# parashardhapola/nabo

Hardware: NVIDIA B200
Metric: target_cells_mapped_per_s (higher is better)
Workload: dtype f64 (candidates: f16x2-split tcgen05, f32 accumulate)

## Files before the change

nabo_b200/csrc/exact.cu:

```cuda
#include <stdarg.h>
#include <stdio.h>

#include "common.cuh"
#include "knn_internal.cuh"
#include "select.cuh"

static thread_local char g_err[512] = "";
int nabo_set_error(int code, const char* fmt, ...) {
    va_list ap;
    va_start(ap, fmt);
    vsnprintf(g_err, sizeof(g_err), fmt, ap);
    va_end(ap);
    return code;
}
extern "C" const char* nabo_last_error(void) { return g_err; }
extern "C" int nabo_abi_version(void) { return NABO_ABI_VERSION; }
extern "C" int nabo_device_check(int* sm_count) {
    int dev = 0;
    NABO_CUDA(cudaGetDevice(&dev));
    cudaDeviceProp p;
    NABO_CUDA(cudaGetDeviceProperties(&p, dev));
    if (sm_count) *sm_count = p.multiProcessorCount;
    if (p.major != 10)
        return nabo_set_error(NABO_EUNSUPPORTED, "device %s is sm_%d%d; this library is built for sm_100a only",
                              p.name, p.major, p.minor);
    return 0;
}

template <int METRIC>
struct Pair {
    static __device__ __forceinline__ double step(double acc, double x, double y, double f) {
        if (METRIC == NABO_EUCLIDEAN) {
            double t = __dsub_rn(x, y);
            return __dadd_rn(acc, __dmul_rn(t, t));
        } else if (METRIC == NABO_MOD_CANBERRA) {
            double absx = fabs(x);
            double num = fabs(__dsub_rn(x, y));
            if (num < __dmul_rn(f, absx)) {
                double den = __dadd_rn(__dadd_rn(absx, fabs(y)), 0.01);
                return __dadd_rn(acc, __ddiv_rn(num, den));
            }
            return __dadd_rn(acc, 1.0);
        } else {
            return __dadd_rn(acc, __dmul_rn(x, y));
        }
    }
    static __device__ __forceinline__ double finish(double acc, double nq, double nr) {
        if (METRIC == NABO_EUCLIDEAN) return __dsqrt_rn(acc);
        if (METRIC == NABO_MOD_CANBERRA) return acc;
        return __dsub_rn(1.0, __ddiv_rn(acc, __dmul_rn(__dsqrt_rn(nq), __dsqrt_rn(nr))));
    }
};

__device__ __forceinline__ double seq_sqnorm(const double* v, int g) {
    double s = 0.0;
    for (int k = 0; k < g; ++k) s = __dadd_rn(s, __dmul_rn(v[k], v[k]));
    return s;
}

constexpr int TQ = 64;
constexpr int TR = 64;
constexpr int NT = 256;
constexpr int LDS_T = TQ + 2;

__device__ __forceinline__ void load_tile_kmajor(double* s, const double* __restrict__ src, int ld,
                                                 int row0, int nrows, int g, const int* row_ids, int k0 = 0) {
    for (int e = threadIdx.x; e < TQ * g; e += NT) {
        int r = e / g, k = e - r * g;
        int row = row0 + r;
        double v = 0.0;
        if (row < nrows) {
            long long rr = row_ids ? row_ids[row] : row;
            v = src[rr * (long long)ld + k0 + k];
        }
        s[k * LDS_T + r] = v;
    }
}

template <int METRIC>
__global__ void __launch_bounds__(NT) dist_tile_kernel(const double* __restrict__ x, int ldx,
                                                       const double* __restrict__ y, int ldy,
                                                       double* __restrict__ d, int ldd, int m, int n,
                                                       int g, double f) {
    extern __shared__ double smem[];
    double* xs = smem;
    double* ys = smem + (size_t)g * LDS_T;
    __shared__ double nqs[TQ], nrs[TR];
    const int q0 = blockIdx.y * TQ, r0 = blockIdx.x * TR;
    load_tile_kmajor(xs, x, ldx, q0, m, g, nullptr);
    load_tile_kmajor(ys, y, ldy, r0, n, g, nullptr);
    __syncthreads();
    if (METRIC == NABO_COSINE) {
        if (threadIdx.x < TQ) {
            double s = 0.0;
            for (int k = 0; k < g; ++k) { double v = xs[k * LDS_T + threadIdx.x]; s = __dadd_rn(s, __dmul_rn(v, v)); }
            nqs[threadIdx.x] = s;
        } else if (threadIdx.x < TQ + TR) {
            int t = threadIdx.x - TQ;
            double s = 0.0;
            for (int k = 0; k < g; ++k) { double v = ys[k * LDS_T + t]; s = __dadd_rn(s, __dmul_rn(v, v)); }
            nrs[t] = s;
        }
        __syncthreads();
    }
    const int tr = threadIdx.x & 15, tq = threadIdx.x >> 4;
    double acc[4][4];
#pragma unroll
    for (int a = 0; a < 4; ++a)
#pragma unroll
        for (int b = 0; b < 4; ++b) acc[a][b] = 0.0;
    for (int k = 0; k < g; ++k) {
        double xv[4], yv[4];
#pragma unroll
        for (int a = 0; a < 4; ++a) xv[a] = xs[k * LDS_T + tq * 4 + a];
#pragma unroll
        for (int b = 0; b < 4; ++b) yv[b] = ys[k * LDS_T + tr * 4 + b];
#pragma unroll
        for (int a = 0; a < 4; ++a)
#pragma unroll
            for (int b = 0; b < 4; ++b) acc[a][b] = Pair<METRIC>::step(acc[a][b], xv[a], yv[b], f);
    }
#pragma unroll
    for (int a = 0; a < 4; ++a) {
        int qi = q0 + tq * 4 + a;
        if (qi >= m) continue;
#pragma unroll
        for (int b = 0; b < 4; ++b) {
            int rj = r0 + tr * 4 + b;
            if (rj < n) {
                double nq = METRIC == NABO_COSINE ? nqs[tq * 4 + a] : 0.0;
                double nr = METRIC == NABO_COSINE ? nrs[tr * 4 + b] : 0.0;
                d[(long long)qi * ldd + rj] = Pair<METRIC>::finish(acc[a][b], nq, nr);
            }
        }
    }
}

template <int METRIC>
static int launch_dist_tiles(const double* x, int ldx, const double* y, int ldy, double* d, int ldd,
                             int m, int n, int g, double f, cudaStream_t s) {
    NABO_ARG(m >= 0 && n >= 0 && g >= 1, "dist: bad shape m=%d n=%d g=%d", m, n, g);
    NABO_ARG(ldx >= g && ldy >= g && ldd >= n, "dist: leading dimension smaller than row length");
    if (m == 0 || n == 0) return 0;
    NABO_ARG(x && y && d, "dist: null pointer");
    size_t smem = 2 * (size_t)g * LDS_T * sizeof(double);
    NABO_ARG(smem <= 200 * 1024, "dist: g=%d exceeds the shared-memory tile (max %d dims)", g,
             (int)(200 * 1024 / (2 * LDS_T * sizeof(double))));
    NABO_CUDA(cudaFuncSetAttribute(dist_tile_kernel<METRIC>, cudaFuncAttributeMaxDynamicSharedMemorySize, (int)smem));
    dim3 grid((n + TR - 1) / TR, (m + TQ - 1) / TQ);
    dist_tile_kernel<METRIC><<<grid, NT, smem, s>>>(x, ldx, y, ldy, d, ldd, m, n, g, f);
    NABO_LAUNCH_CHECK("dist_tile_kernel");
    return 0;
}

extern "C" int nabo_euclidean_dist(const double* x, int ldx, const double* y, int ldy, double* d, int ldd,
                                   int m, int n, int g, void* stream) {
    return launch_dist_tiles<NABO_EUCLIDEAN>(x, ldx, y, ldy, d, ldd, m, n, g, 0.0, (cudaStream_t)stream);
}
extern "C" int nabo_mod_canberra_dist(const double* x, int ldx, const double* y, int ldy, double* d, int ldd,
                                      int m, int n, int g, double f, void* stream) {
    return launch_dist_tiles<NABO_MOD_CANBERRA>(x, ldx, y, ldy, d, ldd, m, n, g, f, (cudaStream_t)stream);
}
extern "C" int nabo_cosine_dist(const double* x, int ldx, const double* y, int ldy, double* d, int ldd,
                                int m, int n, int g, void* stream) {
    return launch_dist_tiles<NABO_COSINE>(x, ldx, y, ldy, d, ldd, m, n, g, 0.0, (cudaStream_t)stream);
}

struct ExactSmem {
    double* xs;
    double* ys;
    double* bd;
    int* bi;
    double* tau_d;
    double* nq;
    double* nr;
    int* tau_i;
    int* cnt;
};

__device__ __forceinline__ ExactSmem carve_exact(double* base, int g, int cap) {
    ExactSmem s;
    s.xs = base;
    s.ys = s.xs + (size_t)g * LDS_T;
    s.bd = s.ys + (size_t)g * LDS_T;
    s.tau_d = s.bd + (size_t)TQ * cap;
    s.nq = s.tau_d + TQ;
    s.nr = s.nq + TQ;
    s.bi = (int*)(s.nr + TR);
    s.tau_i = s.bi + (size_t)TQ * cap;
    s.cnt = s.tau_i + TQ;
    return s;
}
static size_t exact_smem_bytes(int g, int cap) {
    return (2 * (size_t)g * LDS_T + (size_t)TQ * cap + 3 * TQ) * sizeof(double) +
           ((size_t)TQ * cap + 2 * TQ) * sizeof(int);
}

__device__ __forceinline__ void compact_query(const ExactSmem& s, int q, int cap, int ksel, int lane) {
    double* d = s.bd + (size_t)q * cap;
    int* ix = s.bi + (size_t)q * cap;
    int n = s.cnt[q];
    for (int t = n + lane; t < cap; t += 32) { d[t] = CUDART_INF; ix[t] = 0x7fffffff; }
    __syncwarp();
    warp_bitonic_sort(d, ix, cap, lane);
    if (lane == 0) {
        if (n >= ksel) {
            s.cnt[q] = ksel;
            s.tau_d[q] = d[ksel - 1];
            s.tau_i[q] = ix[ksel - 1];
        }
    }
    __syncwarp();
}

template <int METRIC>
__global__ void __launch_bounds__(NT, 1)
knn_exact_kernel(const double* __restrict__ q, int ldq, const double* __restrict__ r, int ldr, int n_query,
                 int n_ref, int g, int k, double f, const uint8_t* __restrict__ mask, int drop_first,
                 int idx_offset, const int* __restrict__ row_ids, const int* __restrict__ n_rows_dev,
                 int cap, int gc, const NaboExactSplit sp, int32_t* __restrict__ out_idx, double* __restrict__ out_dist,
                 const NaboRoute route) {
    extern __shared__ double smem[];
    const ExactSmem s = carve_exact(smem, gc, cap);
    const bool chunked = gc < g;
    const int nq_total = n_rows_dev ? *n_rows_dev : n_query;
    if (sp.mode == 1 && (nq_total > sp.f_max || nq_total <= sp.f_min)) return;
    if (sp.mode == 2 && nq_total <= sp.f_max) return;
    const int r_lo = sp.mode == 1 ? (int)((long long)n_ref * blockIdx.y / sp.nsplit) / TR * TR : 0;
    const int r_hi = sp.mode == 1 ? (blockIdx.y + 1 == (unsigned)sp.nsplit
                                         ? n_ref
                                         : (int)((long long)n_ref * (blockIdx.y + 1) / sp.nsplit) / TR * TR)
                                  : n_ref;
    const int q0 = blockIdx.x * TQ;
    if (q0 >= nq_total) return;
    const int ksel = k + (drop_first ? 1 : 0);
    const int lane = threadIdx.x & 31, warp = threadIdx.x >> 5;
    const int tr = threadIdx.x & 15, tq = threadIdx.x >> 4;

    if (threadIdx.x < TQ) {
        s.cnt[threadIdx.x] = 0;
        s.tau_d[threadIdx.x] = CUDART_INF;
        s.tau_i[threadIdx.x] = 0x7fffffff;
    }
    if (!chunked) {
        load_tile_kmajor(s.xs, q, ldq, q0, nq_total, g, row_ids);
        __syncthreads();
        if (METRIC == NABO_COSINE && threadIdx.x < TQ) {
            double acc = 0.0;
            for (int kk = 0; kk < g; ++kk) { double v = s.xs[kk * LDS_T + threadIdx.x]; acc = __dadd_rn(acc, __dmul_rn(v, v)); }
            s.nq[threadIdx.x] = acc;
        }
    } else if (METRIC == NABO_COSINE) {
        double acc = 0.0;
        for (int kc = 0; kc < g; kc += gc) {
            const int gn = min(gc, g - kc);
            __syncthreads();
            load_tile_kmajor(s.xs, q, ldq, q0, nq_total, gn, row_ids, kc);
            __syncthreads();
            if (threadIdx.x < TQ)
                for (int kk = 0; kk < gn; ++kk) { double v = s.xs[kk * LDS_T + threadIdx.x]; acc = __dadd_rn(acc, __dmul_rn(v, v)); }
        }
        if (threadIdx.x < TQ) s.nq[threadIdx.x] = acc;
    }

    for (int r0 = r_lo; r0 < r_hi; r0 += TR) {
        double acc[4][4];
#pragma unroll
        for (int a = 0; a < 4; ++a)
#pragma unroll
            for (int b = 0; b < 4; ++b) acc[a][b] = 0.0;
        for (int kc = 0; kc < g; kc += gc) {
            const int gn = min(gc, g - kc);
            __syncthreads();
            if (chunked) load_tile_kmajor(s.xs, q, ldq, q0, nq_total, gn, row_ids, kc);
            load_tile_kmajor(s.ys, r, ldr, r0, r_hi, gn, nullptr, kc);
            __syncthreads();
            if (METRIC == NABO_COSINE && threadIdx.x < TR) {
                double nacc = kc == 0 ? 0.0 : s.nr[threadIdx.x];
                for (int kk = 0; kk < gn; ++kk) { double v = s.ys[kk * LDS_T + threadIdx.x]; nacc = __dadd_rn(nacc, __dmul_rn(v, v)); }
                s.nr[threadIdx.x] = nacc;
            }
            if (q0 + tq * 4 < nq_total)
            for (int kk = 0; kk < gn; ++kk) {
                double xv[4], yv[4];
#pragma unroll
                for (int a = 0; a < 4; ++a) xv[a] = s.xs[kk * LDS_T + tq * 4 + a];
#pragma unroll
                for (int b = 0; b < 4; ++b) yv[b] = s.ys[kk * LDS_T + tr * 4 + b];
#pragma unroll
                for (int a = 0; a < 4; ++a)
#pragma unroll
                    for (int b = 0; b < 4; ++b) acc[a][b] = Pair<METRIC>::step(acc[a][b], xv[a], yv[b], f);
            }
        }
        if (METRIC == NABO_COSINE) __syncthreads();
#pragma unroll
        for (int a = 0; a < 4; ++a) {
            const int ql = tq * 4 + a;
            if (q0 + ql >= nq_total) continue;
            const double td = s.tau_d[ql];
            const int ti = s.tau_i[ql];
#pragma unroll
            for (int b = 0; b < 4; ++b) {
                const int j = r0 + tr * 4 + b;
                if (j >= r_hi) continue;
                double d = Pair<METRIC>::finish(acc[a][b], METRIC == NABO_COSINE ? s.nq[ql] : 0.0,
                                                METRIC == NABO_COSINE ? s.nr[tr * 4 + b] : 0.0);
                if (d != d || (mask && mask[j])) d = CUDART_INF;
                if (nabo_less(d, j, td, ti)) {
                    int pos = atomicAdd(&s.cnt[ql], 1);
                    s.bd[(size_t)ql * cap + pos] = d;
                    s.bi[(size_t)ql * cap + pos] = j;
                }
            }
        }
        __syncthreads();
        for (int ql = warp; ql < TQ; ql += NT / 32)
            if (s.cnt[ql] > cap - TR) compact_query(s, ql, cap, ksel, lane);
    }
    __syncthreads();
    for (int ql = warp; ql < TQ; ql += NT / 32) {
        const int qi = q0 + ql;
        if (qi >= nq_total) continue;
        const int n_have = s.cnt[ql];
        {
            double* d = s.bd + (size_t)ql * cap;
            int* ix = s.bi + (size_t)ql * cap;
            for (int t = n_have + lane; t < cap; t += 32) { d[t] = CUDART_INF; ix[t] = 0x7fffffff; }
            __syncwarp();
            warp_bitonic_sort(d, ix, cap, lane);
        }
        if (sp.mode == 1) {
            for (int t = lane; t < ksel; t += 32) {
                const bool have = t < n_have && t < cap;
                const size_t o = ((size_t)blockIdx.y * sp.f_max + qi) * ksel + t;
                sp.part_idx[o] = have ? s.bi[(size_t)ql * cap + t] : -1;
                sp.part_dist[o] = have ? s.bd[(size_t)ql * cap + t] : CUDART_INF;
            }
            continue;
        }
        const long long orow = row_ids ? row_ids[qi] : qi;
        int32_t* oi;
        double* od;
        nabo_route_row(route, orow, k, out_idx, out_dist, oi, od);
        const int skip = drop_first ? 1 : 0;
        for (int t = lane; t < k; t += 32) {
            int src = t + skip;
            int id = -1;
            double dv = CUDART_NAN;
            if (src < n_have && src < cap) {
                id = s.bi[(size_t)ql * cap + src];
                dv = s.bd[(size_t)ql * cap + src];
                if (mask && mask[id]) dv = CUDART_NAN;
                else if (dv == CUDART_INF) {
                    dv = CUDART_NAN;
                }
                id += idx_offset;
            }
            oi[t] = id;
            od[t] = dv;
        }
    }
}

static int exact_cap_for(int ksel) {
    int kp = nabo_next_pow2(ksel);
    int cap = 2 * kp;
    if (cap < 128) cap = 128;
    return cap;
}

__global__ void __launch_bounds__(128)
fallback_merge_kernel(const NaboExactSplit sp, const int* __restrict__ row_ids, const int* __restrict__ n_rows_dev,
                      int k, int drop_first, int idx_offset, const uint8_t* __restrict__ mask, int capp,
                      int32_t* __restrict__ out_idx, double* __restrict__ out_dist, const NaboRoute route) {
    extern __shared__ double smem[];
    const int n_rows = *n_rows_dev;
    if (n_rows > sp.f_max || n_rows <= sp.f_min) return;
    const int lane = threadIdx.x & 31, warp = threadIdx.x >> 5;
    const int qi = blockIdx.x * 4 + warp;
    if (qi >= n_rows) return;
    const int ksel = k + (drop_first ? 1 : 0);
    double* d = smem + (size_t)warp * capp;
    int* ix = (int*)(smem + (size_t)4 * capp) + (size_t)warp * capp;
    const int tot = sp.nsplit * ksel;
    int n_valid = 0;
    for (int c = lane; c < capp; c += 32) {
        double dv = CUDART_INF;
        int id = 0x7fffffff;
        if (c < tot) {
            const int sidx = c / ksel, j = c - sidx * ksel;
            const size_t o = ((size_t)sidx * sp.f_max + qi) * ksel + j;
            const int i0 = sp.part_idx[o];
            if (i0 >= 0) { id = i0; dv = sp.part_dist[o]; ++n_valid; }
        }
        d[c] = dv; ix[c] = id;
    }
    for (int o = 16; o > 0; o >>= 1) n_valid += __shfl_xor_sync(0xffffffffu, n_valid, o);
    __syncwarp();
    warp_bitonic_sort(d, ix, capp, lane);
    const long long orow = row_ids[qi];
    int32_t* oi;
    double* od;
    nabo_route_row(route, orow, k, out_idx, out_dist, oi, od);
    const int skip = drop_first ? 1 : 0;
    for (int t = lane; t < k; t += 32) {
        const int src = t + skip;
        int id = -1;
        double dv = CUDART_NAN;
        if (src < n_valid) {
            id = ix[src];
            dv = d[src];
            if (dv == CUDART_INF || (mask && mask[id])) dv = CUDART_NAN;
            id += idx_offset;
        }
        oi[t] = id;
        od[t] = dv;
    }
}

__global__ void __launch_bounds__(256)
fallback_merge_few_kernel(const NaboExactSplit sp, const int* __restrict__ row_ids, const int* __restrict__ n_rows_dev,
                          int k, int drop_first, int idx_offset, const uint8_t* __restrict__ mask, int capp,
                          int32_t* __restrict__ out_idx, double* __restrict__ out_dist, const NaboRoute route) {
    extern __shared__ double smem[];
    const int n_rows = *n_rows_dev;
    if (n_rows > sp.f_max || n_rows <= sp.f_min) return;
    const int qi = blockIdx.x;
    if (qi >= n_rows) return;
    const int ksel = k + (drop_first ? 1 : 0);
    double* d = smem;
    int* ix = (int*)(smem + capp);
    __shared__ int s_valid;
    if (threadIdx.x == 0) s_valid = 0;
    __syncthreads();
    const int tot = sp.nsplit * ksel;
    int n_valid = 0;
    for (int c = threadIdx.x; c < capp; c += blockDim.x) {
        double dv = CUDART_INF;
        int id = 0x7fffffff;
        if (c < tot) {
            const int sidx = c / ksel, j = c - sidx * ksel;
            const size_t o = ((size_t)sidx * sp.f_max + qi) * ksel + j;
            const int i0 = sp.part_idx[o];
            if (i0 >= 0) { id = i0; dv = sp.part_dist[o]; ++n_valid; }
        }
        d[c] = dv; ix[c] = id;
    }
    atomicAdd(&s_valid, n_valid);
    __syncthreads();
    for (int size = 2; size <= capp; size <<= 1)
        for (int stride = size >> 1; stride > 0; stride >>= 1) {
            for (int t = threadIdx.x; t < (capp >> 1); t += blockDim.x) {
                const int lo = 2 * t - (t & (stride - 1)), hi = lo + stride;
                const bool up = (lo & size) == 0;
                const double dl = d[lo], dh = d[hi];
                const int il = ix[lo], ih = ix[hi];
                if (up ? nabo_less(dh, ih, dl, il) : nabo_less(dl, il, dh, ih)) { d[lo] = dh; d[hi] = dl; ix[lo] = ih; ix[hi] = il; }
            }
            __syncthreads();
        }
    const long long orow = row_ids[qi];
    int32_t* oi;
    double* od;
    nabo_route_row(route, orow, k, out_idx, out_dist, oi, od);
    const int skip = drop_first ? 1 : 0;
    for (int t = threadIdx.x; t < k; t += blockDim.x) {
        const int src = t + skip;
        int id = -1;
        double dv = CUDART_NAN;
        if (src < s_valid) {
            id = ix[src];
            dv = d[src];
            if (dv == CUDART_INF || (mask && mask[id])) dv = CUDART_NAN;
            id += idx_offset;
        }
        oi[t] = id;
        od[t] = dv;
    }
}

int nabo_exact_split_count(int ksel) {
    int s = 2048 / ksel;
    return s > 48 ? 48 : (s < 1 ? 1 : s);
}
size_t nabo_exact_split_workspace(int ksel) {
    (void)ksel;
    return (size_t)2048 * NABO_FALLBACK_SPLIT_ROWS * (sizeof(int32_t) + sizeof(double)) + 512 +
           (size_t)NABO_FALLBACK_FEW_ENTRIES * NABO_FALLBACK_FEW_ROWS * (sizeof(int32_t) + sizeof(double)) + 512;
}

int nabo_knn_exact_fallback(const double* q, int ldq, const double* r, int ldr, int n_query, int n_ref, int g, int k,
                            int metric, double f, const uint8_t* mask, int drop_first, int idx_offset,
                            const int* row_ids, const int* n_rows_dev, void* split_ws, int32_t* out_idx,
                            double* out_dist, const NaboRoute& route, cudaStream_t st) {
    const int ksel = k + (drop_first ? 1 : 0);
    const bool few = n_ref >= NABO_FALLBACK_FEW_MIN_REF;
    if (few) {
        int dev = 0, sms = 148;
        cudaGetDevice(&dev);
        cudaDeviceGetAttribute(&sms, cudaDevAttrMultiProcessorCount, dev);
        NaboExactSplit sf;
        sf.mode = 1;
        sf.nsplit = NABO_FALLBACK_FEW_ENTRIES / ksel < 2 * sms ? NABO_FALLBACK_FEW_ENTRIES / ksel : 2 * sms;
        sf.f_max = NABO_FALLBACK_FEW_ROWS;
        sf.f_min = 0;
        char* base = (char*)split_ws + (size_t)2048 * NABO_FALLBACK_SPLIT_ROWS * (sizeof(int32_t) + sizeof(double)) + 512;
        sf.part_dist = (double*)base;
        sf.part_idx = (int32_t*)(sf.part_dist + (size_t)sf.nsplit * sf.f_max * ksel);
        int rc0 = nabo_knn_exact_launch_ex(q, ldq, r, ldr, NABO_FALLBACK_FEW_ROWS, n_ref, g, ksel, metric, f, mask, 0, 0,
                                           row_ids, n_rows_dev, sf, out_idx, out_dist, route, st);
        if (rc0) return rc0;
        const int cappf = nabo_next_pow2(sf.nsplit * ksel);
        const size_t smf = (size_t)cappf * (sizeof(double) + sizeof(int));
        NABO_CUDA(cudaFuncSetAttribute(fallback_merge_few_kernel, cudaFuncAttributeMaxDynamicSharedMemorySize, (int)smf));
        fallback_merge_few_kernel<<<NABO_FALLBACK_FEW_ROWS, 256, smf, st>>>(sf, row_ids, n_rows_dev, k, drop_first, idx_offset,
                                                                         mask, cappf, out_idx, out_dist, route);
        NABO_LAUNCH_CHECK("fallback_merge_few_kernel");
    }
    NaboExactSplit sp;
    sp.mode = 1;
    sp.nsplit = nabo_exact_split_count(ksel);
    sp.f_max = NABO_FALLBACK_SPLIT_ROWS;
    sp.f_min = few ? NABO_FALLBACK_FEW_ROWS : 0;
    sp.part_dist = (double*)split_ws;
    sp.part_idx = (int32_t*)(sp.part_dist + (size_t)sp.nsplit * sp.f_max * ksel);
    int rc = nabo_knn_exact_launch_ex(q, ldq, r, ldr, NABO_FALLBACK_SPLIT_ROWS, n_ref, g, ksel, metric, f, mask, 0, 0,
                                      row_ids, n_rows_dev, sp, out_idx, out_dist, route, st);
    if (rc) return rc;
    int capp = nabo_next_pow2(sp.nsplit * ksel);
    if (capp < 32) capp = 32;
    const size_t smem = (size_t)4 * capp * (sizeof(double) + sizeof(int));
    NABO_CUDA(cudaFuncSetAttribute(fallback_merge_kernel, cudaFuncAttributeMaxDynamicSharedMemorySize, (int)smem));
    fallback_merge_kernel<<<(NABO_FALLBACK_SPLIT_ROWS + 3) / 4, 128, smem, st>>>(sp, row_ids, n_rows_dev, k, drop_first,
                                                                               idx_offset, mask, capp, out_idx, out_dist,
                                                                               route);
    NABO_LAUNCH_CHECK("fallback_merge_kernel");
    sp.mode = 2;
    return nabo_knn_exact_launch_ex(q, ldq, r, ldr, n_query, n_ref, g, k, metric, f, mask, drop_first, idx_offset,
                                    row_ids, n_rows_dev, sp, out_idx, out_dist, route, st);
}

int nabo_knn_exact_launch(const double* q, int ldq, const double* r, int ldr, int n_query, int n_ref, int g,
                          int k, int metric, double f, const uint8_t* mask, int drop_first, int idx_offset,
                          const int* row_ids, const int* n_rows_dev, int32_t* out_idx, double* out_dist,
                          const NaboRoute& route, cudaStream_t st) {
    NaboExactSplit sp;
    sp.mode = 0; sp.nsplit = 1; sp.f_max = 0; sp.f_min = 0; sp.part_idx = nullptr; sp.part_dist = nullptr;
    return nabo_knn_exact_launch_ex(q, ldq, r, ldr, n_query, n_ref, g, k, metric, f, mask, drop_first, idx_offset,
                                    row_ids, n_rows_dev, sp, out_idx, out_dist, route, st);
}

int nabo_knn_exact_launch_ex(const double* q, int ldq, const double* r, int ldr, int n_query, int n_ref, int g,
                             int k, int metric, double f, const uint8_t* mask, int drop_first, int idx_offset,
                             const int* row_ids, const int* n_rows_dev, const NaboExactSplit& sp, int32_t* out_idx,
                             double* out_dist, const NaboRoute& route, cudaStream_t st) {
    const int ksel = k + (drop_first ? 1 : 0);
    NABO_ARG(k >= 1 && ksel <= 128, "knn: k=%d unsupported (1 <= k, k + drop_first <= 128)", k);
    NABO_ARG(g >= 1, "knn: g=%d", g);
    if (n_query == 0) return 0;
    const int cap = exact_cap_for(ksel);
    int gc = g;
    while (gc > 8 && exact_smem_bytes(gc, cap) > (size_t)227 * 1024) gc = (gc + 1) / 2;
    size_t smem = exact_smem_bytes(gc, cap);
    NABO_ARG(smem <= 227 * 1024, "knn: g=%d with k=%d needs %zu B of shared memory (max 232448)", g, k, smem);
    dim3 grid((n_query + TQ - 1) / TQ, sp.mode == 1 ? sp.nsplit : 1);
#define LAUNCH(M)                                                                                         \
    NABO_CUDA(cudaFuncSetAttribute(knn_exact_kernel<M>, cudaFuncAttributeMaxDynamicSharedMemorySize, (int)smem)); \
    knn_exact_kernel<M><<<grid, NT, smem, st>>>(q, ldq, r, ldr, n_query, n_ref, g, k, f, mask, drop_first, \
                                                idx_offset, row_ids, n_rows_dev, cap, gc, sp, out_idx, out_dist, route);
    if (metric == NABO_EUCLIDEAN) { LAUNCH(NABO_EUCLIDEAN) }
    else if (metric == NABO_MOD_CANBERRA) { LAUNCH(NABO_MOD_CANBERRA) }
    else if (metric == NABO_COSINE) { LAUNCH(NABO_COSINE) }
    else return nabo_set_error(NABO_EINVAL, "knn: unknown metric %d", metric);
#undef LAUNCH
    NABO_LAUNCH_CHECK("knn_exact_kernel");
    return 0;
}

__device__ __forceinline__ double cert_lower_bound(const NaboCert& c, int qi, float tau) {
    if (c.kind == NABO_CERT_LINEAR) return (double)tau - c.c_acc;
    const double sc_inv = c.scal[1], rmax = c.scal[2];
    const double qn2 = c.qn2[qi];
    const double qn = sqrt(qn2);
    const double eps = c.c_acc * (4.0 * qn * rmax + rmax * rmax + qn2);
    const double l2 = (double)tau + qn2 - eps;
    if (!(l2 > 0.0)) return 0.0;
    if (c.kind == NABO_CERT_EUCLID) {
        return sqrt(l2) * sc_inv * (1.0 - 1e-7) - (9.6e-7 * (qn + rmax) + c.abs_slack) * sc_inv;
    }
    double e = sqrt(l2) * sc_inv - 1.0e-6;
    if (!(e > 0.0)) return 0.0;
    return 0.5 * e * e * (1.0 - 1e-9);
}

template <int METRIC, int NU>
__device__ __forceinline__ void pair_rows(const double* __restrict__ x, const double* __restrict__ r, int ldr,
                                          const int* jj, int g, double f, bool vec2, double* acc) {
    const double* y[NU];
#pragma unroll
    for (int u = 0; u < NU; ++u) y[u] = r + (long long)(jj[u] >= 0 ? jj[u] : 0) * ldr;
    double a[NU];
#pragma unroll
    for (int u = 0; u < NU; ++u) a[u] = 0.0;
    int kk = 0;
    if (vec2) {
#pragma unroll 4
        for (; kk + 2 <= g; kk += 2) {
            const double x0 = x[kk], x1 = x[kk + 1];
#pragma unroll
            for (int u = 0; u < NU; ++u) {
                const double2 v = __ldg(reinterpret_cast<const double2*>(y[u] + kk));
                a[u] = Pair<METRIC>::step(a[u], x0, v.x, f);
                a[u] = Pair<METRIC>::step(a[u], x1, v.y, f);
            }
        }
    }
#pragma unroll 4
    for (; kk < g; ++kk) {
        const double xv = x[kk];
#pragma unroll
        for (int u = 0; u < NU; ++u) a[u] = Pair<METRIC>::step(a[u], xv, __ldg(y[u] + kk), f);
    }
#pragma unroll
    for (int u = 0; u < NU; ++u) acc[u] = a[u];
}

#ifdef NABO_RR_STATS
__device__ unsigned long long g_rr_stats[8];
extern "C" int nabo_dbg_rr_stats(unsigned long long* out_host, int reset) {
    cudaDeviceSynchronize();
    cudaMemcpyFromSymbol(out_host, g_rr_stats, sizeof(unsigned long long) * 8);
    if (reset) { unsigned long long z[8] = {0}; cudaMemcpyToSymbol(g_rr_stats, z, sizeof(z)); }
    return 0;
}
#endif
template <int METRIC, bool FROM_BUF>
__global__ void __launch_bounds__(128)
rerank_kernel(const double* __restrict__ q, int ldq, const double* __restrict__ r, int ldr, int n_query,
              int n_ref, int g, int k, double f, const uint8_t* __restrict__ mask, int drop_first,
              int idx_offset, const int32_t* __restrict__ cand, int n_cand, int capp, const NaboCert cert,
              int* __restrict__ fail_rows, int* __restrict__ fail_count,
              int32_t* __restrict__ out_idx, double* __restrict__ out_dist, const NaboRoute route,
              const NaboCandBuf cb, int xs_dims, bool vec2, int row0) {
    extern __shared__ double smem[];
    const int lane = threadIdx.x & 31, warp = threadIdx.x >> 5;
    const int qi = row0 + blockIdx.x * 4 + warp;
    if (qi >= n_query) return;
    int32_t* oi;
    double* od;
    nabo_route_row(route, qi, k, out_idx, out_dist, oi, od);
    double* d = smem + (size_t)warp * capp;
    int* ix = (int*)(smem + (size_t)4 * capp) + (size_t)warp * capp;
    const size_t hist_off = (size_t)6 * capp + (size_t)4 * xs_dims;
    const double* x = q + (long long)qi * ldq;
    double nq = 0.0;
    if (METRIC == NABO_COSINE) nq = seq_sqnorm(x, g);
    int nc = 0;
    float tau_q = CUDART_INF_F;
    if (FROM_BUF) {
        const int n = __ldcg(cb.cnt + qi);
        const unsigned long long* gb = cb.buf + (size_t)qi * sel::CAP;
        float fv[4];
        uint32_t kpl[4];
#pragma unroll
        for (int u = 0; u < 4; ++u) {
            const int i = u * 32 + lane;
            const unsigned long long kv = i < n ? __ldcg(gb + i) : 0ull;
            fv[u] = __uint_as_float((uint32_t)(kv >> 32));
            kpl[u] = (uint32_t)kv;
        }
        uint32_t* hist = reinterpret_cast<uint32_t*>(smem + hist_off) + warp * 256;
        int bin[4], cut_bin, kept;
        bool reach;
        sel::histogram_cut(fv, n, lane, cb.kprime, hist, bin, cut_bin, kept, reach);
        const int c_cut = reach ? (int)hist[cut_bin] : 0;
        const int need = cb.kprime - (kept - c_cut);
#ifdef NABO_RR_STATS
        if (lane == 0) {
            atomicAdd(&g_rr_stats[0], 1ull); atomicAdd(&g_rr_stats[1], (unsigned long long)(reach && c_cut > 48));
            atomicAdd(&g_rr_stats[2], (unsigned long long)c_cut); atomicAdd(&g_rr_stats[3], (unsigned long long)n);
            atomicAdd(&g_rr_stats[4], (unsigned long long)(reach ? c_cut - need : 0));
        }
#endif
        if (!reach || c_cut <= 48) {
            int rank[4] = {0, 0, 0, 0};
            if (reach && c_cut > need) {
#pragma unroll
                for (int us = 0; us < 4; ++us) {
                    unsigned mm = __ballot_sync(0xffffffffu, us * 32 + lane < n && bin[us] == cut_bin);
                    while (mm) {
                        const int src = __ffs(mm) - 1;
                        mm &= mm - 1;
                        const float sv = __shfl_sync(0xffffffffu, fv[us], src);
#pragma unroll
                        for (int u = 0; u < 4; ++u)
                            rank[u] += (sv < fv[u] || (sv == fv[u] && us * 32 + src < u * 32 + lane)) ? 1 : 0;
                    }
                }
                kept = cb.kprime;
            }
            int base = 0;
            float tmax = -CUDART_INF_F;
#pragma unroll
            for (int u = 0; u < 4; ++u) {
                const bool keep = u * 32 + lane < n && (bin[u] < cut_bin || (bin[u] == cut_bin && rank[u] < need));
                const unsigned m = __ballot_sync(0xffffffffu, keep);
                if (keep) {
                    ix[base + __popc(m & ((1u << lane) - 1u))] = (int)kpl[u];
                    tmax = fmaxf(tmax, fv[u]);
                }
                base += __popc(m);
            }
            tmax = sortable_to_float(__reduce_max_sync(0xffffffffu, float_to_sortable(tmax)));
            nc = kept;
            tau_q = reach ? tmax : __ldcg(cb.tau + qi);
        } else {
            uint32_t ks[4];
#pragma unroll
            for (int u = 0; u < 4; ++u) ks[u] = u * 32 + lane < n ? float_to_sortable(fv[u]) : 0xffffffffu;
            sel::sortn(ks, kpl, lane);
            nc = n < cb.kprime ? n : cb.kprime;
            const int e = cb.kprime - 1;
            const uint32_t ts = __shfl_sync(0xffffffffu, (e >> 5) ? ks[1] : ks[0], e & 31);
            tau_q = n >= cb.kprime ? sortable_to_float(ts) : __ldcg(cb.tau + qi);
#pragma unroll
            for (int u = 0; u < 2; ++u)
                if (u * 32 + lane < nc) ix[u * 32 + lane] = (int)kpl[u];
        }
        __syncwarp();
    } else if (cert.kind != NABO_CERT_NONE) {
        tau_q = cert.tau[qi];
    }
    double* xw = xs_dims ? smem + (size_t)4 * capp + (size_t)(4 * capp + 1) / 2 + (size_t)warp * xs_dims : nullptr;
    if (xw) {
        for (int kk = lane; kk < g; kk += 32) xw[kk] = x[kk];
        __syncwarp();
    }
    const double* xq = xw ? xw : x;
    int jj[4];
    int n_slots = 0;
    const bool scramble = (long long)n_ref * ldr * 8 > (96ll << 20);
#pragma unroll
    for (int u = 0; u < 4; ++u) {
        const int c = u * 32 + lane;
        int j = -1;
        if (u * 32 < capp) {
            if (FROM_BUF) {
                const int cpos = scramble ? ((c * 27 + 5) & (capp - 1)) : c;
                j = (u < 2 && cpos < nc) ? ix[cpos] : -1;
            }
            else j = c < n_cand ? cand[(long long)qi * n_cand + c] : -1;
        }
        if (!(j >= 0 && j < n_ref)) j = -1;
        jj[u] = j;
        if (__any_sync(0xffffffffu, j >= 0)) n_slots = u + 1;
    }
    double accs[4] = {0.0, 0.0, 0.0, 0.0};
    if (METRIC == NABO_MOD_CANBERRA) {
#pragma unroll
        for (int u = 0; u < 4; ++u)
            if (u < n_slots) pair_rows<METRIC, 1>(xq, r, ldr, jj + u, g, f, vec2, accs + u);
    } else if (n_slots == 1) pair_rows<METRIC, 1>(xq, r, ldr, jj, g, f, vec2, accs);
    else if (n_slots == 2) pair_rows<METRIC, 2>(xq, r, ldr, jj, g, f, vec2, accs);
    else if (n_slots > 2) pair_rows<METRIC, 4>(xq, r, ldr, jj, g, f, vec2, accs);
    int n_valid = 0, n_finite = 0;
    int ids[4];
#pragma unroll
    for (int u = 0; u < 4; ++u) {
        const int j = jj[u];
        double key = CUDART_INF;
        int id = 0x7fffffff;
        if (j >= 0) {
            double nr = 0.0;
            if (METRIC == NABO_COSINE) nr = seq_sqnorm(r + (long long)j * ldr, g);
            double dv = Pair<METRIC>::finish(accs[u], nq, nr);
            if (dv != dv || (mask && mask[j])) dv = CUDART_INF;
            key = dv;
            id = j;
            ++n_valid;
            n_finite += (dv < CUDART_INF);
        }
        accs[u] = key; ids[u] = id;
    }
    if (capp <= 32) {
        double d1[1] = {accs[0]};
        int i1[1] = {ids[0]};
        warp_bitonic_sort_regs<1>(d1, i1, lane);
        d[lane] = d1[0]; ix[lane] = i1[0];
    } else if (capp <= 64) {
        double d2[2] = {accs[0], accs[1]};
        int i2[2] = {ids[0], ids[1]};
        warp_bitonic_sort_regs<2>(d2, i2, lane);
#pragma unroll
        for (int u = 0; u < 2; ++u) { d[u * 32 + lane] = d2[u]; ix[u * 32 + lane] = i2[u]; }
    } else {
        warp_bitonic_sort_regs<4>(accs, ids, lane);
#pragma unroll
        for (int u = 0; u < 4; ++u) { d[u * 32 + lane] = accs[u]; ix[u * 32 + lane] = ids[u]; }
    }
    __syncwarp();
    for (int o = 16; o > 0; o >>= 1) {
        n_valid += __shfl_xor_sync(0xffffffffu, n_valid, o);
        n_finite += __shfl_xor_sync(0xffffffffu, n_finite, o);
    }
    __syncwarp();
    const int skip = drop_first ? 1 : 0;
    const int ksel = k + skip;
    for (int t = lane; t < k; t += 32) {
        int src = t + skip;
        int id = -1;
        double dv = CUDART_NAN;
        if (src < n_valid) {
            id = ix[src];
            dv = d[src];
            if (dv == CUDART_INF) dv = CUDART_NAN;
            id += idx_offset;
        }
        oi[t] = id;
        od[t] = dv;
    }
    if (cert.kind != NABO_CERT_NONE && lane == 0) {
        const float tau = tau_q;
        bool fail;
        if (tau == CUDART_INF_F) fail = n_valid < n_ref;
        else if (n_finite < ksel) fail = true;
        else fail = !(d[ksel - 1] < cert_lower_bound(cert, qi, tau));
        if (fail) fail_rows[atomicAdd(fail_count, 1)] = qi;
    }
}

int nabo_rerank_launch(const double* q, int ldq, const double* r, int ldr, int n_query, int n_ref, int g, int k,
                       int metric, double f, const uint8_t* mask, int drop_first, int idx_offset,
                       const int32_t* cand, int n_cand, const NaboCert& cert, int* fail_rows, int* fail_count,
                       int32_t* out_idx, double* out_dist, const NaboRoute& route, cudaStream_t st,
                       const NaboCandBuf* from_buf, int row0, bool dependent) {
    NABO_ARG(n_cand >= 1 && n_cand <= 128, "rerank: n_cand=%d unsupported (1..128)", n_cand);
    NABO_ARG(k >= 1 && k + (drop_first ? 1 : 0) <= n_cand, "rerank: k=%d does not fit n_cand=%d", k, n_cand);
    NABO_ARG(row0 >= 0 && row0 <= n_query, "rerank: row0=%d outside [0, %d]", row0, n_query);
    if (n_query - row0 == 0) return 0;
    int capp = nabo_next_pow2(n_cand);
    if (capp < 32) capp = 32;
    size_t smem = (size_t)4 * capp * (sizeof(double) + sizeof(int));
    const int xs_dims = g <= 1024 ? g : 0;
    smem += (size_t)4 * xs_dims * sizeof(double);
    if (from_buf) smem += (size_t)4 * 256 * sizeof(uint32_t);
    const bool vec2 = ((uintptr_t)r & 15) == 0 && (ldr & 1) == 0;
    dim3 grid((n_query - row0 + 3) / 4);
    NaboCandBuf cb;
    cb.buf = nullptr; cb.cnt = nullptr; cb.tau = nullptr; cb.kprime = 0;
    if (from_buf) {
        NABO_ARG(from_buf->kprime >= 1 && from_buf->kprime <= 64 && from_buf->kprime == n_cand,
                 "rerank: buffer mode needs K' = n_cand <= 64");
        cb = *from_buf;
    }
    cudaLaunchConfig_t cfg = {};
    cudaLaunchAttribute attr[1];
    cfg.gridDim = grid; cfg.blockDim = dim3(128); cfg.dynamicSmemBytes = smem; cfg.stream = st;
    attr[0].id = cudaLaunchAttributeProgrammaticStreamSerialization;
    attr[0].val.programmaticStreamSerializationAllowed = 1;
    cfg.attrs = attr; cfg.numAttrs = dependent ? 1 : 0;
#define LAUNCH(M)                                                                                              \
    if (from_buf)                                                                                              \
        NABO_CUDA(cudaLaunchKernelEx(&cfg, rerank_kernel<M, true>, q, ldq, r, ldr, n_query, n_ref, g, k, f, mask, \
                                     drop_first, idx_offset, cand, n_cand, capp, cert, fail_rows, fail_count,  \
                                     out_idx, out_dist, route, cb, xs_dims, vec2, row0));                      \
    else                                                                                                       \
        NABO_CUDA(cudaLaunchKernelEx(&cfg, rerank_kernel<M, false>, q, ldq, r, ldr, n_query, n_ref, g, k, f, mask, \
                                     drop_first, idx_offset, cand, n_cand, capp, cert, fail_rows, fail_count,  \
                                     out_idx, out_dist, route, cb, xs_dims, vec2, row0));
    if (metric == NABO_EUCLIDEAN) { LAUNCH(NABO_EUCLIDEAN) }
    else if (metric == NABO_MOD_CANBERRA) { LAUNCH(NABO_MOD_CANBERRA) }
    else if (metric == NABO_COSINE) { LAUNCH(NABO_COSINE) }
    else return nabo_set_error(NABO_EINVAL, "rerank: unknown metric %d", metric);
#undef LAUNCH
    NABO_LAUNCH_CHECK("rerank_kernel");
    return 0;
}

extern "C" int nabo_rerank_exact(const double* q, int ldq, const double* r, int ldr, int n_query, int n_ref,
                                 int g, int k, int metric, double dist_factor, const uint8_t* ref_mask,
                                 int drop_first, int idx_offset, const int32_t* cand, int n_cand,
                                 int32_t* out_idx, double* out_dist, void* stream) {
    NABO_ARG(q && r && cand && out_idx && out_dist, "rerank: null pointer");
    NABO_ARG(ldq >= g && ldr >= g, "rerank: leading dimension smaller than g");
    NaboCert none;
    none.kind = NABO_CERT_NONE; none.tau = nullptr; none.qn2 = nullptr; none.scal = nullptr; none.c_acc = 0.0; none.abs_slack = 0.0;
    NaboRoute plain;
    plain.n_parts = 0;
    return nabo_rerank_launch(q, ldq, r, ldr, n_query, n_ref, g, k, metric, dist_factor, ref_mask, drop_first,
                              idx_offset, cand, n_cand, none, nullptr, nullptr, out_idx, out_dist, plain,
                              (cudaStream_t)stream);
}
```

nabo_b200/csrc/fast.cu:

```cuda
#include "knn_internal.cuh"

static const double kCAcc = 1.52587890625e-05;

static size_t cb_extra_bytes(int n_query, int n_ref, int g) {
    const size_t a = nabo_cb_extra_bytes(n_ref, g), b = nabo_cbs_extra_bytes(n_query, n_ref, g);
    return a > b ? a : b;
}

size_t nabo_fast_workspace_bytes(int n_query, int n_ref, int g, int k, int metric) {
    if (metric == NABO_MOD_CANBERRA)
        return nabo_align_up((size_t)n_query * nabo_cb_kprime(k, 1) * 4 * NABO_CBS_MAX_SPLIT, 256) +
               (2 + NABO_CBS_MAX_SPLIT) * nabo_align_up((size_t)n_query * 4, 256) +
               nabo_align_up(nabo_cb_pretile_floats(n_query, g) * 4, 256) + nabo_align_up(nabo_cb_pretile_floats(n_ref, g) * 4, 256) +
               nabo_align_up(nabo_exact_split_workspace(k + 1), 256) + nabo_align_up(cb_extra_bytes(n_query, n_ref, g), 256) + 4096;
    return nabo_tc_workspace_bytes(n_query, n_ref, g, k, 1) + nabo_align_up((size_t)n_query * 4, 256) +
           nabo_align_up(nabo_exact_split_workspace(k + 1), 256) + 1024;
}

int nabo_knn_fast(const double* q, int ldq, const double* r, int ldr, int n_query, int n_ref, int g, int k,
                  int metric, double f, const uint8_t* mask, int drop_first, int idx_offset, int32_t* out_idx,
                  double* out_dist, const NaboRoute& route, void* workspace, size_t workspace_bytes,
                  int64_t* stats_host, cudaStream_t st) {
    NaboStageTimer tm(stats_host != nullptr, st);
    tm.begin();
    const bool use_tc = (metric == NABO_EUCLIDEAN || metric == NABO_COSINE) && nabo_tc_supported(g, k, drop_first) &&
                        n_ref > nabo_tc_kprime(k, drop_first);
    const bool use_cb = metric == NABO_MOD_CANBERRA && nabo_cb_supported(g, k, drop_first) &&
                        n_ref > nabo_cb_kprime(k, drop_first);
    if (use_cb) {
        if (workspace_bytes < nabo_fast_workspace_bytes(n_query, n_ref, g, k, metric))
            return nabo_set_error(NABO_EWORKSPACE, "knn: workspace too small");
        NaboArena ar(workspace, workspace_bytes);
        const int kprime = nabo_cb_kprime(k, drop_first);
        const bool sliced_ok = nabo_cbs_supported(g, k, drop_first) && f >= 1e-6;
        const int n_split = sliced_ok ? nabo_cbs_split(n_query, n_ref, k, drop_first) : 1;
        int32_t* cand = ar.take<int32_t>((size_t)n_query * kprime * n_split);
        float* tau = ar.take<float>((size_t)n_query * n_split);
        int* fail_rows = ar.take<int>(n_query);
        int* fail_count = ar.take<int>(1);
        float* qt = ar.take<float>(nabo_cb_pretile_floats(n_query, g));
        float* rt = ar.take<float>(nabo_cb_pretile_floats(n_ref, g));
        char* split_ws = ar.take<char>(nabo_exact_split_workspace(k + (drop_first ? 1 : 0)));
        char* extra = ar.take<char>(cb_extra_bytes(n_query, n_ref, g));
        if (!ar.ok) return nabo_set_error(NABO_EWORKSPACE, "knn: workspace too small");
        NABO_CUDA(cudaMemsetAsync(fail_count, 0, sizeof(int), st));
        const bool sliced = sliced_ok;
        int rc = sliced
                     ? nabo_cbs_candidates(q, ldq, r, ldr, n_query, n_ref, g, k, f, mask, drop_first, n_split, rt, extra,
                                           cb_extra_bytes(n_query, n_ref, g), cand, tau, st)
                     : nabo_cb_candidates(q, ldq, r, ldr, n_query, n_ref, g, k, f, mask, drop_first, qt, rt, extra, cand,
                                          tau, st);
        if (rc) return rc;
        if (n_split > 1) {
            rc = nabo_tau_min_launch(tau, n_query, n_split, st);
            if (rc) return rc;
        }
        tm.end(0);
        NaboCert cert;
        cert.kind = NABO_CERT_LINEAR; cert.tau = tau; cert.qn2 = nullptr; cert.scal = nullptr; cert.c_acc = nabo_cb_eps(g); cert.abs_slack = 0.0;
        rc = nabo_rerank_launch(q, ldq, r, ldr, n_query, n_ref, g, k, metric, f, mask, drop_first, idx_offset, cand,
                                kprime * n_split, cert, fail_rows, fail_count, out_idx, out_dist, route, st);
        if (rc) return rc;
        tm.end(1);
        rc = nabo_knn_exact_fallback(q, ldq, r, ldr, n_query, n_ref, g, k, metric, f, mask, drop_first, idx_offset,
                                     fail_rows, fail_count, split_ws, out_idx, out_dist, route, st);
        if (rc) return rc;
        tm.end(2);
        if (stats_host) {
            int nfail = 0;
            NABO_CUDA(cudaMemcpyAsync(&nfail, fail_count, sizeof(int), cudaMemcpyDeviceToHost, st));
            NABO_CUDA(cudaStreamSynchronize(st));
            stats_host[0] = n_query; stats_host[1] = nfail; stats_host[2] = kprime;
            stats_host[3] = sliced ? 10 : 11;
            stats_host[4] = tm.ns(0); stats_host[5] = tm.ns(1); stats_host[6] = tm.ns(2);
        }
        return 0;
    }
    if (!use_tc) {
        int rc = nabo_knn_exact_launch(q, ldq, r, ldr, n_query, n_ref, g, k, metric, f, mask, drop_first, idx_offset,
                                       nullptr, nullptr, out_idx, out_dist, route, st);
        tm.end(0);
        if (rc) return rc;
        if (stats_host) {
            NABO_CUDA(cudaStreamSynchronize(st));
            stats_host[1] = n_query;
            stats_host[3] = 1;
            stats_host[4] = tm.ns(0);
        }
        return 0;
    }
    if (workspace_bytes < nabo_fast_workspace_bytes(n_query, n_ref, g, k, metric))
        return nabo_set_error(NABO_EWORKSPACE, "knn: workspace too small (%zu < %zu)", workspace_bytes,
                              nabo_fast_workspace_bytes(n_query, n_ref, g, k, metric));
    NaboArena ar(workspace, workspace_bytes);
    int32_t* cand = nullptr;
    float* tau = nullptr;
    double *qn2 = nullptr, *scal = nullptr;
    int kprime = 0, launches = 0;
    NaboCandBuf raw;
    raw.buf = nullptr;
    int n_split = nabo_tc_split(n_query, n_ref, g);
    while (n_split > 1 && n_split * nabo_tc_kprime(k, drop_first) > 128) --n_split;
    int* fail_rows = ar.take<int>(n_query);
    int* fail_count = ar.take<int>(1);
    char* split_ws = ar.take<char>(nabo_exact_split_workspace(k + (drop_first ? 1 : 0)));
    if (!ar.ok) return nabo_set_error(NABO_EWORKSPACE, "knn: workspace too small");
    NABO_CUDA(cudaMemsetAsync(fail_count, 0, sizeof(int), st));
    NaboTailSplit tail;
    tail.rows_full = 0; tail.applies = 0;
    tail.dry = stats_host != nullptr;
    int rc = nabo_tc_candidates(q, ldq, r, ldr, n_query, n_ref, g, k, metric, mask, drop_first, &n_split, ar, &cand,
                                &kprime, &tau, &qn2, &scal, &launches, tm, st, &raw, &tail);
    if (rc) return rc;
    if (!ar.ok) return nabo_set_error(NABO_EWORKSPACE, "knn: workspace too small");
    NaboCert cert;
    cert.kind = metric == NABO_COSINE ? NABO_CERT_COSINE : NABO_CERT_EUCLID;
    cert.tau = tau; cert.qn2 = qn2; cert.scal = scal; cert.c_acc = kCAcc;
    cert.abs_slack = 2.0 * sqrt((double)g) * 5.9604644775390625e-08;
    int row0 = 0;
    if (tail.rows_full > 0) {
        rc = nabo_rerank_launch(q, ldq, r, ldr, tail.rows_full, n_ref, g, k, metric, f, mask, drop_first, idx_offset, cand,
                                kprime * n_split, cert, fail_rows, fail_count, out_idx, out_dist, route, st, &raw, 0, true);
        if (rc) return rc;
        tm.end(0);
        row0 = tail.rows_full;
    }
    launches += tail.applies;
    rc = nabo_rerank_launch(q, ldq, r, ldr, n_query, n_ref, g, k, metric, f, mask, drop_first, idx_offset, cand,
                            kprime * n_split, cert, fail_rows, fail_count, out_idx, out_dist, route, st,
                            raw.buf ? &raw : nullptr, row0);
    if (rc) return rc;
    tm.end(1);
    rc = nabo_knn_exact_fallback(q, ldq, r, ldr, n_query, n_ref, g, k, metric, f, mask, drop_first, idx_offset,
                                 fail_rows, fail_count, split_ws, out_idx, out_dist, route, st);
    if (rc) return rc;
    tm.end(2);
    if (stats_host) {
        int nfail = 0;
        NABO_CUDA(cudaMemcpyAsync(&nfail, fail_count, sizeof(int), cudaMemcpyDeviceToHost, st));
        NABO_CUDA(cudaStreamSynchronize(st));
        stats_host[0] = n_query;
        stats_host[1] = nfail;
        stats_host[2] = kprime;
        stats_host[3] = launches + 4;
        stats_host[4] = tm.ns(0);
        stats_host[5] = tm.ns(1);
        stats_host[6] = tm.ns(2);
        stats_host[7] = tm.ns(3);
    }
    return 0;
}
```

nabo_b200/csrc/knn_internal.cuh:

```cuda
#pragma once
#include "common.cuh"

#define NABO_MAX_PARTS 16
struct NaboRoute {
    int n_parts;
    int bounds[NABO_MAX_PARTS + 1];
    int32_t* idx[NABO_MAX_PARTS];
    double* dist[NABO_MAX_PARTS];
};
__device__ __forceinline__ void nabo_route_row(const NaboRoute& rt, long long row, int k, int32_t* out_idx,
                                               double* out_dist, int32_t*& ri, double*& rd) {
    if (rt.n_parts == 0) {
        ri = out_idx + row * k;
        rd = out_dist + row * k;
        return;
    }
    int p = 0;
    while (p + 1 < rt.n_parts && row >= rt.bounds[p + 1]) ++p;
    const long long local = row - rt.bounds[p];
    ri = rt.idx[p] + local * k;
    rd = rt.dist[p] + local * k;
}

#define NABO_FALLBACK_SPLIT_ROWS 2048
#define NABO_FALLBACK_FEW_ROWS 64
#define NABO_FALLBACK_FEW_ENTRIES 16384
#define NABO_FALLBACK_FEW_MIN_REF 262144
struct NaboExactSplit {
    int mode;
    int nsplit, f_max, f_min;
    int32_t* part_idx;
    double* part_dist;
};
int nabo_exact_split_count(int ksel);
size_t nabo_exact_split_workspace(int ksel);
int nabo_knn_exact_launch_ex(const double* q, int ldq, const double* r, int ldr, int n_query, int n_ref, int g,
                             int k, int metric, double f, const uint8_t* mask, int drop_first, int idx_offset,
                             const int* row_ids, const int* n_rows_dev, const NaboExactSplit& sp, int32_t* out_idx,
                             double* out_dist, const NaboRoute& route, cudaStream_t st);
int nabo_knn_exact_fallback(const double* q, int ldq, const double* r, int ldr, int n_query, int n_ref, int g, int k,
                            int metric, double f, const uint8_t* mask, int drop_first, int idx_offset,
                            const int* row_ids, const int* n_rows_dev, void* split_ws, int32_t* out_idx,
                            double* out_dist, const NaboRoute& route, cudaStream_t st);

int nabo_knn_exact_launch(const double* q, int ldq, const double* r, int ldr, int n_query, int n_ref, int g,
                          int k, int metric, double f, const uint8_t* mask, int drop_first, int idx_offset,
                          const int* row_ids, const int* n_rows_dev, int32_t* out_idx, double* out_dist,
                          const NaboRoute& route, cudaStream_t st);

#define NABO_CERT_NONE 0
#define NABO_CERT_EUCLID 1
#define NABO_CERT_COSINE 2
#define NABO_CERT_LINEAR 3
struct NaboCert {
    int kind;
    const float* tau;
    const double* qn2;
    const double* scal;
    double c_acc;
    double abs_slack;
};

struct NaboCandBuf {
    const unsigned long long* buf;
    const int* cnt;
    const float* tau;
    int kprime;
};
int nabo_rerank_launch(const double* q, int ldq, const double* r, int ldr, int n_query, int n_ref, int g, int k,
                       int metric, double f, const uint8_t* mask, int drop_first, int idx_offset,
                       const int32_t* cand, int n_cand, const NaboCert& cert, int* fail_rows, int* fail_count,
                       int32_t* out_idx, double* out_dist, const NaboRoute& route, cudaStream_t st,
                       const NaboCandBuf* from_buf = nullptr, int row0 = 0, bool dependent = false);

struct NaboTailSplit {
    int dry;
    int rows_full;
    int applies;
};

struct NaboStageTimer;
bool nabo_tc_supported(int g, int k, int drop_first);
int nabo_tc_kprime(int k, int drop_first);
size_t nabo_tc_workspace_bytes(int n_query, int n_ref, int g, int k, int drop_first);
#define NABO_TC_MAX_SPLIT 3
int nabo_tc_split(int n_query, int n_ref, int g);
int nabo_tc_candidates(const double* q, int ldq, const double* r, int ldr, int n_query, int n_ref, int g, int k,
                       int metric, const uint8_t* mask, int drop_first, int* n_split_io, NaboArena& ar, int32_t** cand_idx_out,
                       int* kprime_out, float** cert_tau_out, double** qn2_out, double** scal_out, int* launches,
                       NaboStageTimer& tm, cudaStream_t st, NaboCandBuf* raw_out = nullptr, NaboTailSplit* tail = nullptr);

bool nabo_cb_supported(int g, int k, int drop_first);
int nabo_cb_kprime(int k, int drop_first);
double nabo_cb_eps(int g);
size_t nabo_cb_pretile_floats(int n, int g);
size_t nabo_cb_extra_bytes(int n_ref, int g);
int nabo_cb_candidates(const double* q, int ldq, const double* r, int ldr, int n_query, int n_ref, int g, int k,
                       double f, const uint8_t* mask, int drop_first, float* qt, float* rt, void* extra, int32_t* cand,
                       float* tau, cudaStream_t st);

int nabo_cb_pretile_launch(const double* x, int ld, int n, int g, float* out, cudaStream_t st);
bool nabo_cbs_supported(int g, int k, int drop_first);
size_t nabo_cbs_extra_bytes(int n_query, int n_ref, int g);
#define NABO_CBS_MAX_SPLIT 3
int nabo_cbs_split(int n_query, int n_ref, int k, int drop_first);
int nabo_cbs_candidates(const double* q, int ldq, const double* r, int ldr, int n_query, int n_ref, int g, int k,
                        double f, const uint8_t* mask, int drop_first, int n_split, float* rt, void* extra,
                        size_t extra_bytes, int32_t* cand, float* tau, cudaStream_t st);
int nabo_tau_min_launch(float* tau, int n_query, int n_split, cudaStream_t st);

size_t nabo_fast_workspace_bytes(int n_query, int n_ref, int g, int k, int metric);
int nabo_knn_fast(const double* q, int ldq, const double* r, int ldr, int n_query, int n_ref, int g, int k,
                  int metric, double f, const uint8_t* mask, int drop_first, int idx_offset, int32_t* out_idx,
                  double* out_dist, const NaboRoute& route, void* workspace, size_t workspace_bytes,
                  int64_t* stats_host, cudaStream_t st);

struct NaboStageTimer {
    static constexpr int MAXS = 4;
    bool on;
    cudaStream_t st;
    cudaEvent_t start;
    cudaEvent_t stop[MAXS];
    int prev[MAXS];
    bool used[MAXS];
    int last;
    NaboStageTimer(bool enable, cudaStream_t s) : on(enable), st(s), last(-1) {
        for (int i = 0; i < MAXS; ++i) { prev[i] = -1; used[i] = false; }
        if (on) {
            cudaEventCreate(&start);
            for (int i = 0; i < MAXS; ++i) cudaEventCreate(&stop[i]);
        }
    }
    ~NaboStageTimer() {
        if (on) {
            cudaEventDestroy(start);
            for (int i = 0; i < MAXS; ++i) cudaEventDestroy(stop[i]);
        }
    }
    void begin() { if (on) cudaEventRecord(start, st); }
    void end(int i) {
        if (!on) return;
        cudaEventRecord(stop[i], st);
        used[i] = true;
        prev[i] = last;
        last = i;
    }
    long long ns(int i) {
        if (!on || !used[i]) return 0;
        float ms = 0.f;
        cudaEventElapsedTime(&ms, prev[i] < 0 ? start : stop[prev[i]], stop[i]);
        return (long long)((double)ms * 1e6);
    }
};
```

nabo_b200/csrc/select.cuh:

```cuda
#pragma once
#include "common.cuh"

namespace sel {

constexpr int CAP = 128;
constexpr int KPL = CAP / 32;

__device__ __forceinline__ unsigned long long make_key(float score, uint32_t col) {
    return ((unsigned long long)__float_as_uint(score) << 32) | col;
}

__device__ __forceinline__ void cex(uint32_t& s0, uint32_t& p0, uint32_t& s1, uint32_t& p1, bool up) {
    const bool sw = up ? (s1 < s0) : (s0 < s1);
    if (sw) { uint32_t t = s0; s0 = s1; s1 = t; t = p0; p0 = p1; p1 = t; }
}

__device__ __forceinline__ void sortn(uint32_t (&s)[KPL], uint32_t (&pl)[KPL], int lane) {
#pragma unroll
    for (int size = 2; size <= 32 * KPL; size <<= 1) {
#pragma unroll
        for (int stride = size >> 1; stride > 0; stride >>= 1) {
            if (stride >= 32) {
                const int du = stride >> 5;
#pragma unroll
                for (int u = 0; u < KPL; ++u) {
                    if ((u & du) == 0) {
                        const bool up = (((u * 32) & size) == 0);
                        cex(s[u], pl[u], s[u | du], pl[u | du], up);
                    }
                }
            } else {
#pragma unroll
                for (int u = 0; u < KPL; ++u) {
                    const int i = u * 32 + lane;
                    const uint32_t os = __shfl_xor_sync(0xffffffffu, s[u], stride);
                    const uint32_t op = __shfl_xor_sync(0xffffffffu, pl[u], stride);
                    const bool up = ((i & size) == 0);
                    const bool lower = ((lane & stride) == 0);
                    const bool take_min = (up == lower);
                    const bool other = take_min ? (os < s[u]) : (s[u] < os);
                    if (other) { s[u] = os; pl[u] = op; }
                }
            }
        }
    }
}

__device__ __forceinline__ void compact_sort_inline(unsigned long long* gbuf, int n, int lane, int kprime,
                                                    uint32_t (&s)[KPL], uint32_t (&pl)[KPL], int& nc, float& nt) {
    __syncwarp();
#pragma unroll
    for (int u = 0; u < KPL; ++u) {
        const int i = u * 32 + lane;
        const unsigned long long kv = i < n ? __ldcg(gbuf + i) : 0ull;
        s[u] = i < n ? float_to_sortable(__uint_as_float((uint32_t)(kv >> 32))) : 0xffffffffu;
        pl[u] = (uint32_t)kv;
    }
    sortn(s, pl, lane);
    nc = n < kprime ? n : kprime;
#pragma unroll
    for (int u = 0; u < KPL; ++u) {
        const int i = u * 32 + lane;
        if (i < nc) gbuf[i] = ((unsigned long long)__float_as_uint(sortable_to_float(s[u])) << 32) | pl[u];
    }
    const int e = kprime - 1;
    uint32_t ts = s[0];
#pragma unroll
    for (int u = 1; u < KPL; ++u)
        if ((e >> 5) == u) ts = s[u];
    ts = __shfl_sync(0xffffffffu, ts, e & 31);
    nt = n >= kprime ? sortable_to_float(ts) : CUDART_INF_F;
    __syncwarp();
}

static __device__ __noinline__ void compact_sort(unsigned long long* gbuf, int n, int lane, int kprime, int& nc, float& nt) {
    uint32_t s[KPL], pl[KPL];
    compact_sort_inline(gbuf, n, lane, kprime, s, pl, nc, nt);
}

static __device__ __noinline__ void compact_select(unsigned long long* gbuf, int n, int lane, int kprime, int max_keep,
                                            uint32_t* hist, int& nc, float& nt) {
    __syncwarp();
    float fv[KPL];
    uint32_t pl[KPL];
    float flo = CUDART_INF_F, fhi = -CUDART_INF_F;
#pragma unroll
    for (int u = 0; u < KPL; ++u) {
        const int i = u * 32 + lane;
        const unsigned long long kv = i < n ? __ldcg(gbuf + i) : 0ull;
        fv[u] = __uint_as_float((uint32_t)(kv >> 32));
        pl[u] = (uint32_t)kv;
        if (i < n) { flo = fminf(flo, fv[u]); fhi = fmaxf(fhi, fv[u]); }
    }
    flo = sortable_to_float(__reduce_min_sync(0xffffffffu, float_to_sortable(flo)));
    fhi = sortable_to_float(__reduce_max_sync(0xffffffffu, float_to_sortable(fhi)));
    reinterpret_cast<uint4*>(hist)[lane * 2] = make_uint4(0, 0, 0, 0);
    reinterpret_cast<uint4*>(hist)[lane * 2 + 1] = make_uint4(0, 0, 0, 0);
    __syncwarp();
    const float range = fhi - flo;
    const float scale = range > 0.f ? 255.999f / range : 0.f;
    int bin[KPL];
#pragma unroll
    for (int u = 0; u < KPL; ++u) {
        const int i = u * 32 + lane;
        bin[u] = max(0, min(255, (int)((fv[u] - flo) * scale)));
        if (i < n) atomicAdd(&hist[bin[u]], 1u);
    }
    __syncwarp();
    const uint4 h0 = reinterpret_cast<const uint4*>(hist)[lane * 2];
    const uint4 h1 = reinterpret_cast<const uint4*>(hist)[lane * 2 + 1];
    const uint32_t c[8] = {h0.x, h0.y, h0.z, h0.w, h1.x, h1.y, h1.z, h1.w};
    uint32_t mine = 0;
#pragma unroll
    for (int e = 0; e < 8; ++e) mine += c[e];
    uint32_t incl = mine;
#pragma unroll
    for (int o = 1; o < 32; o <<= 1) {
        const uint32_t v = __shfl_up_sync(0xffffffffu, incl, o);
        if (lane >= o) incl += v;
    }
    const unsigned reach = __ballot_sync(0xffffffffu, incl >= (uint32_t)kprime);
    int cut_bin = 255;
    uint32_t kept = (uint32_t)n;
    if (reach) {
        const int owner = __ffs(reach) - 1;
        uint32_t run = incl - mine;
        int b = 7;
        uint32_t k_at = 0;
        bool found = false;
#pragma unroll
        for (int e = 0; e < 8; ++e) {
            run += c[e];
            if (!found && run >= (uint32_t)kprime) { found = true; b = e; k_at = run; }
        }
        cut_bin = __shfl_sync(0xffffffffu, lane * 8 + b, owner);
        kept = __shfl_sync(0xffffffffu, k_at, owner);
    }
    if ((int)kept > max_keep) {
        compact_sort(gbuf, n, lane, kprime, nc, nt);
        return;
    }
    uint32_t base = 0;
    float tmax = -CUDART_INF_F;
#pragma unroll
    for (int u = 0; u < KPL; ++u) {
        const int i = u * 32 + lane;
        const bool keep = i < n && bin[u] <= cut_bin;
        const unsigned m = __ballot_sync(0xffffffffu, keep);
        if (keep) {
            gbuf[base + __popc(m & ((1u << lane) - 1u))] = ((unsigned long long)__float_as_uint(fv[u]) << 32) | pl[u];
            tmax = fmaxf(tmax, fv[u]);
        }
        base += __popc(m);
    }
    tmax = sortable_to_float(__reduce_max_sync(0xffffffffu, float_to_sortable(tmax)));
    nc = (int)kept;
    nt = reach ? tmax : CUDART_INF_F;
    __syncwarp();
}

__device__ __forceinline__ void histogram_cut(const float (&fv)[KPL], int n, int lane, int kprime, uint32_t* hist,
                                              int (&bin)[KPL], int& cut_bin, int& kept, bool& reach_out) {
    float flo = CUDART_INF_F, fhi = -CUDART_INF_F;
#pragma unroll
    for (int u = 0; u < KPL; ++u)
        if (u * 32 + lane < n) { flo = fminf(flo, fv[u]); fhi = fmaxf(fhi, fv[u]); }
    flo = sortable_to_float(__reduce_min_sync(0xffffffffu, float_to_sortable(flo)));
    fhi = sortable_to_float(__reduce_max_sync(0xffffffffu, float_to_sortable(fhi)));
    reinterpret_cast<uint4*>(hist)[lane * 2] = make_uint4(0, 0, 0, 0);
    reinterpret_cast<uint4*>(hist)[lane * 2 + 1] = make_uint4(0, 0, 0, 0);
    __syncwarp();
    const float range = fhi - flo;
    const float scale = range > 0.f ? 255.999f / range : 0.f;
#pragma unroll
    for (int u = 0; u < KPL; ++u) {
        bin[u] = max(0, min(255, (int)((fv[u] - flo) * scale)));
        if (u * 32 + lane < n) atomicAdd(&hist[bin[u]], 1u);
    }
    __syncwarp();
    const uint4 h0 = reinterpret_cast<const uint4*>(hist)[lane * 2];
    const uint4 h1 = reinterpret_cast<const uint4*>(hist)[lane * 2 + 1];
    const uint32_t c[8] = {h0.x, h0.y, h0.z, h0.w, h1.x, h1.y, h1.z, h1.w};
    uint32_t mine = 0;
#pragma unroll
    for (int e = 0; e < 8; ++e) mine += c[e];
    uint32_t incl = mine;
#pragma unroll
    for (int o = 1; o < 32; o <<= 1) {
        const uint32_t v = __shfl_up_sync(0xffffffffu, incl, o);
        if (lane >= o) incl += v;
    }
    const unsigned reach = __ballot_sync(0xffffffffu, incl >= (uint32_t)kprime);
    cut_bin = 255;
    kept = n;
    reach_out = reach != 0;
    if (reach) {
        const int owner = __ffs(reach) - 1;
        uint32_t run = incl - mine;
        int b = 7;
        uint32_t k_at = 0;
        bool found = false;
#pragma unroll
        for (int e = 0; e < 8; ++e) {
            run += c[e];
            if (!found && run >= (uint32_t)kprime) { found = true; b = e; k_at = run; }
        }
        cut_bin = __shfl_sync(0xffffffffu, lane * 8 + b, owner);
        kept = (int)__shfl_sync(0xffffffffu, k_at, owner);
    }
    __syncwarp();
}

}
```

nabo_b200/csrc/tc_candidates.cu:

```cuda
#include "common.cuh"
#include "knn_internal.cuh"
#include "ptx.cuh"
#include "select.cuh"

#include <cuda_fp16.h>

namespace tc {

constexpr int TILE = 128;
constexpr int NTHREADS = 512;
constexpr int MAX_G = 128;
constexpr int PRODUCER_WARP = 12;
constexpr int MMA_WARP = 13;
constexpr int TMEM_WARP = 12;
constexpr int KPL = 4;
constexpr int CAP = 32 * KPL;
static_assert(CAP == sel::CAP, "the fused re-rank (exact.cu) reads the candidate buffers with sel::CAP keys per query");
constexpr int CHUNK = 32;
constexpr int MAX_KPRIME = 96;
constexpr int SLEEP_NS = 2000;
constexpr int NACC = 4;
constexpr int MAX_STAGES = 4;
constexpr uint32_t KSTEP_BYTES = TILE * 16 * 2;

__host__ __device__ inline int kp_for(int g) { return (3 * g + 3 + 15) / 16 * 16; }
__host__ __device__ inline size_t tile_bytes(int kp) { return (size_t)TILE * kp * 2; }

struct SmemPlan {
    int nq;
    int slab;
    int stages;
    size_t stage_bytes;
    size_t a_off, b_off, sort_off, bar_off, total;
};
inline SmemPlan plan_smem(int g) {
    const int kp = kp_for(g);
    const size_t bars = 512;
    const size_t budget = 227 * 1024 - 1024;
    auto room = [&](int nq) {
        const size_t used = nq * tile_bytes(kp) + (size_t)4 * nq * 256 * 4 + bars;
        return budget > used ? budget - used : (size_t)0;
    };
    SmemPlan p;
    p.nq = 3;
    p.slab = 0;
    p.stage_bytes = tile_bytes(kp);
    p.stages = (int)(room(3) / p.stage_bytes);
    if (p.stages > MAX_STAGES) p.stages = MAX_STAGES;
    if (p.stages < 2) {
        p.nq = 2;
        p.stages = 0;
        for (int slab = 4; slab >= 2 && g <= MAX_G; slab /= 2) {
            const size_t sb = (size_t)slab * KSTEP_BYTES;
            int st = (int)(room(2) / sb);
            if (st > MAX_STAGES) st = MAX_STAGES;
            if (st >= 2 && st * sb > p.stages * p.stage_bytes) { p.slab = slab; p.stages = st; p.stage_bytes = sb; }
        }
    }
    const size_t a = p.nq * tile_bytes(kp);
    p.a_off = 0;
    p.b_off = a;
    p.sort_off = a + (size_t)p.stages * p.stage_bytes;
    p.bar_off = p.sort_off + (size_t)4 * p.nq * 256 * 4;
    p.total = p.bar_off + bars;
    return p;
}

__global__ void __launch_bounds__(256)
norms_kernel(const double* __restrict__ x, int ld, int n, int g, double* __restrict__ norms2,
             unsigned int* __restrict__ maxn2_bits) {
    int row = blockIdx.x * blockDim.x + threadIdx.x;
    float mine = 0.f;
    if (row < n) {
        const double* p = x + (long long)row * ld;
        double s = 0.0;
        for (int k = 0; k < g; ++k) s = fma(p[k], p[k], s);
        norms2[row] = s;
        if (isfinite(s)) mine = __double2float_ru(s);
    }
    for (int o = 16; o > 0; o >>= 1) mine = fmaxf(mine, __shfl_xor_sync(0xffffffffu, mine, o));
    if ((threadIdx.x & 31) == 0 && mine > 0.f) atomicMax(maxn2_bits, __float_as_uint(mine));
}

__global__ void scale_kernel(const unsigned int* __restrict__ maxq_bits, const unsigned int* __restrict__ maxr_bits,
                             int cosine, double* __restrict__ scal) {
    double sc = 1.0, rmax;
    if (cosine) {
        sc = 32.0;
        rmax = 32.0 * (1.0 + 1e-6);
    } else {
        float mq = __uint_as_float(*maxq_bits), mr = __uint_as_float(*maxr_bits);
        double mx = sqrt((double)fmaxf(mq, mr));
        if (mx > 0.0 && isfinite(mx)) {
            int e;
            frexp(mx, &e);
            sc = ldexp(1.0, 6 - e);
        }
        rmax = sqrt((double)__uint_as_float(*maxr_bits)) * sc * (1.0 + 1e-6);
    }
    scal[0] = sc;
    scal[1] = 1.0 / sc;
    scal[2] = rmax;
    scal[3] = cosine ? 1.0 : 0.0;
}

constexpr int PACK_SPLIT = 4;
template <bool IS_QUERY>
__global__ void __launch_bounds__(TILE * PACK_SPLIT)
pack_kernel(const double* __restrict__ x, int ld, int n, int g, int kp, const double* __restrict__ norms2,
            const double* __restrict__ scal, const uint8_t* __restrict__ mask, __half* __restrict__ out,
            double* __restrict__ qn2_out) {
    __shared__ double part[PACK_SPLIT][TILE];
    const int r = threadIdx.x & (TILE - 1);
    const int c = threadIdx.x / TILE;
    const long long row = (long long)blockIdx.x * TILE + r;
    __half* tile = out + (size_t)blockIdx.x * TILE * kp;
    const bool live = row < n;
    const double sc = scal[0];
    const bool cosine = scal[3] != 0.0;
    double mul = sc;
    bool dead = false;
    if (live && cosine) {
        double nn = sqrt(norms2[row]);
        if (nn > 0.0 && isfinite(nn)) mul = sc / nn; else { mul = 0.0; dead = true; }
    }
    if (live && !IS_QUERY && mask && mask[row]) dead = true;
    if (!live && !IS_QUERY) dead = true;
    const double* p = x + (live ? row : 0) * (long long)ld;
    const int nchunks = kp / 8;
    auto chunk = [&](int kc, double& n2, double n2_row) {
        __align__(16) __half h[8];
#pragma unroll
        for (int e = 0; e < 8; ++e) {
            const int col = kc * 8 + e;
            __half v = __float2half(0.f);
            if (live && col < 3 * g) {
                const int seg = col / g, k = col - seg * g;
                const double xv = p[k] * mul;
                const __half hi = __double2half(xv);
                const __half lo = __double2half(xv - (double)__half2float(hi));
                if (seg == 0) { const double t = (double)__half2float(hi) + (double)__half2float(lo); n2 = fma(t, t, n2); }
                if (IS_QUERY) {
                    const __half src = seg == 2 ? lo : hi;
                    v = __float2half(-2.0f * __half2float(src));
                } else {
                    v = seg == 1 ? lo : hi;
                }
            } else if (live && col < 3 * g + 3) {
                if (IS_QUERY) v = __float2half(1.0f);
            }
            h[e] = v;
        }
        if (!IS_QUERY && (live || dead) && 3 * g + 3 > kc * 8 && 3 * g < kc * 8 + 8) {
            double rem = dead ? 60000.0 : n2_row;
            for (int t = 0; t < 3; ++t) {
                const int col = 3 * g + t;
                const __half piece = __double2half(rem);
                rem -= (double)__half2float(piece);
                if (dead && t > 0) { if (col >= kc * 8 && col < kc * 8 + 8) h[col - kc * 8] = __float2half(0.f); continue; }
                if (col >= kc * 8 && col < kc * 8 + 8) h[col - kc * 8] = piece;
            }
        }
        *reinterpret_cast<uint4*>(reinterpret_cast<char*>(tile) + (size_t)kc * (TILE * 16) + (r >> 3) * 128 + (r & 7) * 16) =
            *reinterpret_cast<const uint4*>(h);
    };
    const int norm_lo = (3 * g) / 8, norm_hi = (3 * g + 2) / 8;
    double n2 = 0.0;
    for (int kc = c; kc < nchunks; kc += PACK_SPLIT) {
        if (!IS_QUERY && kc >= norm_lo && kc <= norm_hi) continue;
        chunk(kc, n2, 0.0);
    }
    if (!IS_QUERY) {
        for (int kc = norm_lo + c; kc <= norm_hi && kc < nchunks; kc += PACK_SPLIT)
            for (int e = 0; e < 8; ++e) {
                const int col = kc * 8 + e;
                if (live && col < g) {
                    const double xv = p[col] * mul;
                    const __half hi = __double2half(xv);
                    const __half lo = __double2half(xv - (double)__half2float(hi));
                    const double t = (double)__half2float(hi) + (double)__half2float(lo);
                    n2 = fma(t, t, n2);
                }
            }
    }
    part[c][r] = n2;
    __syncthreads();
    double n2_row = part[0][r];
#pragma unroll
    for (int i = 1; i < PACK_SPLIT; ++i) n2_row += part[i][r];
    if (!IS_QUERY) {
        for (int kc = norm_lo + c; kc <= norm_hi && kc < nchunks; kc += PACK_SPLIT) {
            double unused = 0.0;
            chunk(kc, unused, n2_row);
        }
    }
    if (IS_QUERY && c == 0 && live && qn2_out) qn2_out[row] = n2_row;
}

struct Params {
    const __half* qa;
    const __half* rb;
    int n_query, n_ref, kp, n_items, n_rtiles, stages, kprime, kc_out, soft;
    int signal_round;
    int n_split;
    unsigned long long* cand_buf;
    int* cand_cnt;
    float* cand_tau;
    int32_t* cand_idx;
    float* cert_tau;
    size_t a_off, b_off, sort_off, bar_off;
};

struct Barriers {
    uint64_t a_full, a_empty;
    uint64_t b_full[MAX_STAGES], b_empty[MAX_STAGES];
    uint64_t acc_full[NACC], acc_empty[NACC];
    uint32_t tmem_base;
};

using namespace sel;

#ifdef NABO_TC_STATS
__device__ unsigned long long g_tc_stats[12];
#define TC_STAT(i, v) (tc_loc[i] += (unsigned long long)(v))
#define TC_CLK(var) const long long var = clock64()
#define TC_CLK_ADD(i, t0) (tc_loc[i] += (unsigned long long)(clock64() - (t0)))
#define TC_DECL unsigned long long tc_loc[12] = {0, 0, 0, 0, 0, 0, 0, 0, 0, 0, 0, 0}
#define TC_FLUSH do { if ((threadIdx.x & 31) == 0) for (int i_ = 0; i_ < 12; ++i_) { if (tc_loc[i_]) atomicAdd(&g_tc_stats[i_], tc_loc[i_]); tc_loc[i_] = 0; } } while (0)
#define TC_ARG , unsigned long long (&tc_loc)[12]
#define TC_PASS , tc_loc
#else
#define TC_STAT(i, v)
#define TC_CLK(var)
#define TC_CLK_ADD(i, t0)
#define TC_DECL
#define TC_FLUSH
#define TC_ARG
#define TC_PASS
#endif

__device__ __forceinline__ void filter_chunk(const uint32_t (&vr)[32], uint32_t col0, float tau,
                                             unsigned long long* mybuf, int& cnt TC_ARG) {
    float v[32];
#pragma unroll
    for (int i = 0; i < 32; ++i) v[i] = __uint_as_float(vr[i]);
    float g4[4];
#pragma unroll
    for (int gi = 0; gi < 4; ++gi) {
        const float a = ptx::min3(v[8 * gi], v[8 * gi + 1], v[8 * gi + 2]);
        const float b = ptx::min3(v[8 * gi + 3], v[8 * gi + 4], v[8 * gi + 5]);
        g4[gi] = ptx::min3(a, b, fminf(v[8 * gi + 6], v[8 * gi + 7]));
    }
    const float m = fminf(fminf(g4[0], g4[1]), fminf(g4[2], g4[3]));
#ifdef NABO_TC_STATS
    {
        const unsigned hb = __ballot_sync(0xffffffffu, m < tau);
        if ((threadIdx.x & 31) == 0) { TC_STAT(0, 1); if (hb) { TC_STAT(1, 1); TC_STAT(2, __popc(hb)); } }
        int na = 0;
        for (int i = 0; i < 32; ++i) na += v[i] < tau;
        for (int o = 16; o > 0; o >>= 1) na += __shfl_xor_sync(0xffffffffu, na, o);
        if ((threadIdx.x & 31) == 0) TC_STAT(3, na);
    }
#endif
    if (m < tau) {
#pragma unroll
        for (int gi = 0; gi < 4; ++gi) {
            if (g4[gi] < tau) {
#pragma unroll
                for (int i = 0; i < 8; ++i) {
                    if (v[8 * gi + i] < tau) {
                        NABO_DEV_ASSERT(cnt >= 0 && cnt < CAP);
                        mybuf[cnt] = make_key(v[8 * gi + i], col0 + 8 * gi + i);
                        ++cnt;
                    }
                }
            }
        }
    }
}

template <bool SPLIT>
__device__ __forceinline__ bool work_piece(const Params& p, int c, int r, int& slot, int& qitem, int& j0, int& j1) {
    slot = c + r * (int)gridDim.x;
    if (!SPLIT) {
        if (slot >= p.n_items) return false;
        qitem = slot; j0 = 0; j1 = p.n_rtiles;
        return true;
    }
    if (slot >= p.n_items * p.n_split) return false;
    qitem = slot / p.n_split;
    const int seg = slot - qitem * p.n_split;
    j0 = (int)((long long)p.n_rtiles * seg / p.n_split);
    j1 = (int)((long long)p.n_rtiles * (seg + 1) / p.n_split);
    return true;
}

template <int KSTEPS, bool SPLIT, int NQ = 3, int SLAB = 0>
__global__ void __launch_bounds__(NTHREADS, 1) candidates_kernel(const Params p) {
    static_assert(NQ * 4 <= PRODUCER_WARP && (SLAB == 0 || KSTEPS == 0), "tile plan");
    constexpr int N_EPI_WARPS = 4 * NQ;
    extern __shared__ __align__(1024) uint8_t smem[];
    Barriers* bars = reinterpret_cast<Barriers*>(smem + p.bar_off);
    const int warp = threadIdx.x >> 5, lane = threadIdx.x & 31;
    const int ksteps = p.kp / 16;
    const uint32_t a_tile_bytes = (uint32_t)tile_bytes(p.kp);
    const int nslab = SLAB ? (ksteps + SLAB - 1) / SLAB : 1;
    const uint32_t stage_bytes = SLAB ? SLAB * KSTEP_BYTES : a_tile_bytes;

    if (threadIdx.x == 0) {
        ptx::mbar_init(&bars->a_full, 1);
        ptx::mbar_init(&bars->a_empty, 1);
        for (int s = 0; s < MAX_STAGES; ++s) { ptx::mbar_init(&bars->b_full[s], 1); ptx::mbar_init(&bars->b_empty[s], 1); }
        for (int q = 0; q < NACC; ++q) { ptx::mbar_init(&bars->acc_full[q], 1); ptx::mbar_init(&bars->acc_empty[q], 4); }
        ptx::fence_barrier_init();
    }
    if (warp == TMEM_WARP) ptx::tmem_alloc(&bars->tmem_base, 512);
    ptx::tc_fence_before();
    __syncthreads();
    ptx::tc_fence_after();
    const uint32_t tmem_base = bars->tmem_base;

    if (warp == PRODUCER_WARP) {
        if (lane == 0) {
            uint32_t t = 0, it = 0;
            for (int wr = 0;; ++wr, ++it) {
                int w, item, j0, j1;
                if (!work_piece<SPLIT>(p, blockIdx.x, wr, w, item, j0, j1)) break;
                ptx::mbar_wait_hint(&bars->a_empty, (it & 1) ^ 1, SLEEP_NS);
                ptx::mbar_arrive_expect_tx(&bars->a_full, NQ * a_tile_bytes);
                for (int q = 0; q < NQ; ++q) {
                    const char* src = reinterpret_cast<const char*>(p.qa) + (size_t)(item * NQ + q) * a_tile_bytes;
                    char* dst = reinterpret_cast<char*>(smem + p.a_off) + (size_t)q * a_tile_bytes;
                    for (uint32_t o = 0; o < a_tile_bytes; o += 8192)
                        ptx::bulk_g2s(dst + o, src + o, min(8192u, a_tile_bytes - o), &bars->a_full);
                }
                for (int j = j0; j < j1; ++j)
                    for (int sl = 0; sl < nslab; ++sl, ++t) {
                        const uint32_t s = t % p.stages, use = t / p.stages;
                        const uint32_t off = sl * stage_bytes, bytes = min(stage_bytes, a_tile_bytes - off);
                        ptx::mbar_wait_hint(&bars->b_empty[s], (use & 1) ^ 1, SLEEP_NS);
                        ptx::mbar_arrive_expect_tx(&bars->b_full[s], bytes);
                        const char* src = reinterpret_cast<const char*>(p.rb) + (size_t)j * a_tile_bytes + off;
                        char* dst = reinterpret_cast<char*>(smem + p.b_off) + (size_t)s * stage_bytes;
                        for (uint32_t o = 0; o < bytes; o += 8192)
                            ptx::bulk_g2s(dst + o, src + o, min(8192u, bytes - o), &bars->b_full[s]);
                    }
            }
        }
    } else if (warp == MMA_WARP) {
        {
            const uint32_t idesc = ptx::make_idesc_f16(TILE, TILE);
            const uint32_t lbo = TILE * 16, sbo = 128;
            const uint64_t ad0 = ptx::make_smem_desc(ptx::smem_u32(smem + p.a_off), lbo, sbo);
            const uint64_t bd0 = ptx::make_smem_desc(ptx::smem_u32(smem + p.b_off), lbo, sbo);
            uint32_t t = 0, it = 0, n = 0;
            for (int wr = 0;; ++wr, ++it) {
                int w, item, j0, j1;
                if (!work_piece<SPLIT>(p, blockIdx.x, wr, w, item, j0, j1)) break;
                ptx::mbar_wait(&bars->a_full, it & 1);
                for (int j = j0; j < j1; ++j, n += NQ, ++t)
                    for (int sl = 0; sl < nslab; ++sl) {
                        const uint32_t u = t * nslab + sl, s = u % p.stages, use = u / p.stages;
                        ptx::mbar_wait(&bars->b_full[s], use & 1);
                        const uint64_t bd1 = bd0 + (uint64_t)((s * stage_bytes) >> 4);
                        const int k0 = sl * SLAB;
#pragma unroll
                        for (int q = 0; q < NQ; ++q) {
                            const uint32_t job = n + q, buf = job & 3;
                            if (sl == 0) {
                                ptx::mbar_wait(&bars->acc_empty[buf], ((job >> 2) & 1) ^ 1);
                                ptx::tc_fence_after();
                            }
                            const uint32_t d_tmem = tmem_base + buf * TILE;
                            const uint64_t ad1 = ad0 + (uint64_t)((q * a_tile_bytes + k0 * KSTEP_BYTES) >> 4);
                            if (ptx::elect_one()) {
                                if (SLAB > 0) {
#pragma unroll
                                    for (int ks = 0; ks < SLAB; ++ks)
                                        if (k0 + ks < ksteps)
                                            ptx::mma_f16_ss(d_tmem, ad1 + ks * ((2 * lbo) >> 4), bd1 + ks * ((2 * lbo) >> 4),
                                                            idesc, k0 + ks > 0 ? 1u : 0u);
                                } else if (KSTEPS > 0) {
#pragma unroll
                                    for (int ks = 0; ks < KSTEPS; ++ks)
                                        ptx::mma_f16_ss(d_tmem, ad1 + ks * ((2 * lbo) >> 4), bd1 + ks * ((2 * lbo) >> 4), idesc,
                                                        ks > 0 ? 1u : 0u);
                                } else {
                                    for (int ks = 0; ks < ksteps; ++ks)
                                        ptx::mma_f16_ss(d_tmem, ad1 + ks * ((2 * lbo) >> 4), bd1 + ks * ((2 * lbo) >> 4), idesc,
                                                        ks > 0 ? 1u : 0u);
                                }
                                if (sl == nslab - 1) ptx::mma_commit(&bars->acc_full[buf]);
                                if (q == NQ - 1) {
                                    ptx::mma_commit(&bars->b_empty[s]);
                                    if (j == j1 - 1 && sl == nslab - 1) ptx::mma_commit(&bars->a_empty);
                                }
                            }
                            __syncwarp();
                        }
                    }
            }
        }
    } else if (warp < N_EPI_WARPS) {
        const int q = warp >> 2;
        const int quarter = warp & 3;
        const int row = quarter * 32 + lane;
        const int slot = q * TILE + row;
        const uint32_t tlane0 = tmem_base + ((uint32_t)(quarter * 32) << 16);
        uint32_t t = 0;
        uint32_t* hist = reinterpret_cast<uint32_t*>(smem + p.sort_off) + (size_t)warp * 256;
        TC_DECL;
        for (int wr = 0;; ++wr) {
            int w, item, j0, j1;
            if (!work_piece<SPLIT>(p, blockIdx.x, wr, w, item, j0, j1)) break;
            unsigned long long* mybuf = p.cand_buf + ((size_t)w * NQ * TILE + slot) * CAP;
            float tau = CUDART_INF_F;
            int cnt = 0;
            TC_CLK(t_item);
            for (int j = j0; j < j1; ++j, ++t) {
                const uint32_t job = t * NQ + q, buf = job & 3, acc_par = (job >> 2) & 1;
                const uint32_t taddr0 = tlane0 + buf * TILE;
                TC_CLK(t_w);
                ptx::mbar_wait(&bars->acc_full[buf], acc_par);
                ptx::tc_fence_after();
                TC_CLK_ADD(7, t_w);
                NABO_DEV_ASSERT(j >= 0 && j < p.n_rtiles);
                auto compact_over = [&](int lim) {
                    unsigned need = __ballot_sync(0xffffffffu, cnt > lim);
                    TC_CLK(t_c);
                    while (need) {
                        const int src = __ffs(need) - 1;
                        need &= need - 1;
                        unsigned long long* gb = reinterpret_cast<unsigned long long*>(
                            __shfl_sync(0xffffffffu, (unsigned long long)mybuf, src));
                        const int n = __shfl_sync(0xffffffffu, cnt, src);
                        int nc;
                        float nt;
                        compact_select(gb, n, lane, p.kprime, p.soft - 8, hist, nc, nt);
                        if (lane == src) { cnt = nc; tau = nt; }
                        if (lane == 0) TC_STAT(4, 1);
                    }
                    TC_CLK_ADD(5, t_c);
                };
#pragma unroll 1
                for (int c = 0; c < TILE / CHUNK; ++c) {
                    uint32_t vr[32];
                    TC_CLK(t_l);
                    ptx::tmem_ld_32x32(taddr0 + c * CHUNK, vr);
                    ptx::tmem_ld_wait();
                    TC_CLK_ADD(8, t_l);
                    if (c == TILE / CHUNK - 1) {
                        ptx::tc_fence_before();
                        __syncwarp();
                        if (lane == 0) ptx::mbar_arrive(&bars->acc_empty[buf]);
                    }
                    TC_CLK(t_f);
                    filter_chunk(vr, (uint32_t)(j * TILE + c * CHUNK), tau, mybuf, cnt TC_PASS);
                    TC_CLK_ADD(6, t_f);
                    compact_over(c == TILE / CHUNK - 1 ? p.soft : CAP - CHUNK);
                }
            }
            TC_CLK(t_e);
            p.cand_cnt[(size_t)w * NQ * TILE + slot] = cnt;
            p.cand_tau[(size_t)w * NQ * TILE + slot] = tau;
            TC_CLK_ADD(9, t_e);
            TC_CLK_ADD(10, t_item);
            TC_FLUSH;
            if (!SPLIT && p.signal_round == wr + 1) {
                __threadfence();
                asm volatile("bar.sync 1, %0;" ::"n"(N_EPI_WARPS * 32) : "memory");
                if (threadIdx.x == 0) asm volatile("griddepcontrol.launch_dependents;" ::: "memory");
            }
        }
    }
    ptx::tc_fence_before();
    __syncthreads();
    if (warp == TMEM_WARP) ptx::tmem_dealloc(tmem_base, 512);
}

template <int NQ>
__global__ void __launch_bounds__(256)
emit_kernel(const Params p) {
    const int lane = threadIdx.x & 31;
    const long long wq = (long long)blockIdx.x * 8 + (threadIdx.x >> 5);
    if (wq >= (long long)p.n_items * p.n_split * NQ * TILE) return;
    const int w = (int)(wq / (NQ * TILE)), slot = (int)(wq - (long long)w * NQ * TILE);
    const int item = w / p.n_split, seg = w - item * p.n_split;
    const long long qg = (long long)item * NQ * TILE + slot;
    if (qg >= p.n_query) return;
    const int n = p.cand_cnt[wq];
    const float old_tau = p.cand_tau[wq];
    NABO_DEV_ASSERT(n >= 0 && n <= CAP);
    uint32_t ks[KPL], kpl[KPL];
    int nc;
    float nt;
    compact_sort_inline(p.cand_buf + (size_t)wq * CAP, n, lane, p.kprime, ks, kpl, nc, nt);
#pragma unroll
    for (int u = 0; u < 4; ++u) {
        const int i = u * 32 + lane;
        if (i < p.kc_out) {
            int32_t id = -1;
            if (i < nc && kpl[u] < (uint32_t)p.n_ref) id = (int32_t)kpl[u];
            p.cand_idx[(qg * p.n_split + seg) * p.kc_out + i] = id;
        }
    }
    if (lane == 0) p.cert_tau[(long long)seg * p.n_query + qg] = n >= p.kprime ? nt : old_tau;
}

}

bool nabo_tc_supported(int g, int k, int drop_first) {
    if (g < 1 || g > tc::MAX_G) return false;
    const tc::SmemPlan pl = tc::plan_smem(g);
    const int ksel = k + (drop_first ? 1 : 0);
    return pl.stages >= 2 && ksel + 8 <= tc::MAX_KPRIME;
}

int nabo_tc_kprime(int k, int drop_first) {
    const int ksel = k + (drop_first ? 1 : 0);
    int kprime = ksel + (ksel / 4 > 8 ? ksel / 4 : 8);
    if (kprime > tc::MAX_KPRIME) kprime = tc::MAX_KPRIME;
    return kprime;
}

static int tc_grid(int n_items) {
    int dev = 0, sms = 148;
    cudaGetDevice(&dev);
    cudaDeviceGetAttribute(&sms, cudaDevAttrMultiProcessorCount, dev);
    return n_items < sms ? n_items : sms;
}

int nabo_tc_split(int n_query, int n_ref, int g) {
    const int nq = tc::plan_smem(g).nq;
    const int n_items = (n_query + nq * tc::TILE - 1) / (nq * tc::TILE);
    const int n_rtiles = (n_ref + tc::TILE - 1) / tc::TILE;
    int s = n_items > 0 ? tc_grid(1 << 30) / n_items : 1;
    if (s > NABO_TC_MAX_SPLIT) s = NABO_TC_MAX_SPLIT;
    while (s > 1 && n_rtiles / s < 32) --s;
    return s < 1 ? 1 : s;
}

__global__ void tau_min_kernel(float* __restrict__ tau, int n_query, int n_split) {
    const int i = blockIdx.x * blockDim.x + threadIdx.x;
    if (i >= n_query) return;
    float t = tau[i];
    for (int s = 1; s < n_split; ++s) t = fminf(t, tau[(size_t)s * n_query + i]);
    tau[i] = t;
}

int nabo_tau_min_launch(float* tau, int n_query, int n_split, cudaStream_t st) {
    tau_min_kernel<<<(n_query + 255) / 256, 256, 0, st>>>(tau, n_query, n_split);
    NABO_LAUNCH_CHECK("tau_min_kernel");
    return 0;
}

size_t nabo_tc_workspace_bytes(int n_query, int n_ref, int g, int k, int drop_first) {
    const int kp = tc::kp_for(g);
    const size_t tb = tc::tile_bytes(kp);
    const int nq = tc::plan_smem(g).nq;
    const int n_items = (n_query + nq * tc::TILE - 1) / (nq * tc::TILE);
    const int n_rtiles = (n_ref + tc::TILE - 1) / tc::TILE;
    const int kprime = nabo_tc_kprime(k, drop_first);
    size_t b = 0;
    b += nabo_align_up((size_t)n_items * nq * tb, 256);
    b += nabo_align_up((size_t)n_rtiles * tb, 256);
    b += nabo_align_up((size_t)n_query * 8, 256) * 2;
    b += nabo_align_up((size_t)n_ref * 8, 256);
    b += nabo_align_up((size_t)n_items * NABO_TC_MAX_SPLIT * nq * tc::TILE * (tc::CAP * 8 + 8), 256) + 512;
    b += nabo_align_up((size_t)n_query * kprime * 4 * NABO_TC_MAX_SPLIT, 256);
    b += nabo_align_up((size_t)n_query * 4 * NABO_TC_MAX_SPLIT, 256) + nabo_align_up((size_t)n_query * 4, 256);
    b += 4096;
    return b;
}

int nabo_tc_candidates(const double* q, int ldq, const double* r, int ldr, int n_query, int n_ref, int g, int k,
                       int metric, const uint8_t* mask, int drop_first, int* n_split_io, NaboArena& ar, int32_t** cand_idx_out,
                       int* kprime_out, float** cert_tau_out, double** qn2_out, double** scal_out, int* launches,
                       NaboStageTimer& tm, cudaStream_t st, NaboCandBuf* raw_out, NaboTailSplit* tail) {
    int n_split = *n_split_io;
    const int kp = tc::kp_for(g);
    const tc::SmemPlan pl = tc::plan_smem(g);
    const size_t tb = tc::tile_bytes(kp);
    const int n_items = (n_query + pl.nq * tc::TILE - 1) / (pl.nq * tc::TILE);
    const int n_qtiles = n_items * pl.nq;
    const int n_rtiles = (n_ref + tc::TILE - 1) / tc::TILE;
    const int kprime = nabo_tc_kprime(k, drop_first);
    if (n_split < 1 || n_split > NABO_TC_MAX_SPLIT) n_split = 1;
    const int grid = tc_grid(n_items * n_split);

    __half* qa = (__half*)ar.take<char>((size_t)n_qtiles * tb);
    __half* rb = (__half*)ar.take<char>((size_t)n_rtiles * tb);
    double* qnorm = ar.take<double>(n_query);
    double* qn2 = ar.take<double>(n_query);
    double* rnorm = ar.take<double>(n_ref);
    const size_t n_slots = (size_t)n_items * n_split * pl.nq * tc::TILE;
    unsigned long long* cbuf = ar.take<unsigned long long>(n_slots * tc::CAP);
    int* ccnt = ar.take<int>(n_slots);
    float* ctau = ar.take<float>(n_slots);
    int32_t* cand = ar.take<int32_t>((size_t)n_query * kprime * n_split);
    float* tau = ar.take<float>((size_t)n_query * n_split);
    double* scal = ar.take<double>(4);
    unsigned int* maxbits = ar.take<unsigned int>(2);
    if (!ar.ok) return nabo_set_error(NABO_EWORKSPACE, "knn: workspace too small for the tensor-core pass");

    NABO_CUDA(cudaMemsetAsync(maxbits, 0, 2 * sizeof(unsigned int), st));
    tc::norms_kernel<<<(n_query + 255) / 256, 256, 0, st>>>(q, ldq, n_query, g, qnorm, maxbits);
    tc::norms_kernel<<<(n_ref + 255) / 256, 256, 0, st>>>(r, ldr, n_ref, g, rnorm, maxbits + 1);
    tc::scale_kernel<<<1, 1, 0, st>>>(maxbits, maxbits + 1, metric == NABO_COSINE ? 1 : 0, scal);
    tc::pack_kernel<true><<<n_qtiles, tc::TILE * tc::PACK_SPLIT, 0, st>>>(q, ldq, n_query, g, kp, qnorm, scal, nullptr, qa, qn2);
    tc::pack_kernel<false><<<n_rtiles, tc::TILE * tc::PACK_SPLIT, 0, st>>>(r, ldr, n_ref, g, kp, rnorm, scal, mask, rb, nullptr);
    NABO_LAUNCH_CHECK("tc pack kernels");
    tm.end(3);

    tc::Params p;
    p.qa = qa; p.rb = rb;
    p.n_query = n_query; p.n_ref = n_ref; p.kp = kp; p.n_items = n_items; p.n_rtiles = n_rtiles;
    p.stages = pl.stages; p.kprime = kprime; p.kc_out = kprime; p.n_split = n_split;
    p.cand_buf = cbuf; p.cand_cnt = ccnt; p.cand_tau = ctau; p.cand_idx = cand; p.cert_tau = tau;
    p.a_off = pl.a_off; p.b_off = pl.b_off; p.sort_off = pl.sort_off; p.bar_off = pl.bar_off;
    p.soft = tc::CAP - tc::CHUNK - 16 > kprime ? tc::CAP - tc::CHUNK - 16 : kprime;
    const bool fused = raw_out && n_split == 1 && kprime <= 64;
    const int rem_items = n_items % grid;
    const bool tail_applies = tail && fused && n_items > grid && rem_items > 0 && grid - rem_items >= 16;
    const bool overlap = tail_applies && !tail->dry;
    p.signal_round = overlap ? n_items / grid : 0;
    if (tail) {
        tail->applies = tail_applies ? 1 : 0;
        tail->rows_full = overlap ? (n_items - rem_items) * pl.nq * tc::TILE : 0;
    }
#define NABO_TC_LAUNCH1(KS, SPLIT, NQ, SLAB)                                                                       \
    do {                                                                                                           \
        NABO_CUDA(cudaFuncSetAttribute(tc::candidates_kernel<KS, SPLIT, NQ, SLAB>,                                 \
                                       cudaFuncAttributeMaxDynamicSharedMemorySize, (int)pl.total));               \
        tc::candidates_kernel<KS, SPLIT, NQ, SLAB><<<grid, tc::NTHREADS, pl.total, st>>>(p);                       \
    } while (0)
#define NABO_TC_LAUNCH(KS, NQ, SLAB)                                                                               \
    do {                                                                                                           \
        if (n_split > 1) NABO_TC_LAUNCH1(KS, true, NQ, SLAB);                                                      \
        else NABO_TC_LAUNCH1(KS, false, NQ, SLAB);                                                                 \
    } while (0)
    if (pl.stages < 2) return nabo_set_error(NABO_EUNSUPPORTED, "knn: g=%d outside the tensor-core tile plans", g);
    if (pl.nq == 2) {
        if (pl.slab == 4) NABO_TC_LAUNCH(0, 2, 4);
        else NABO_TC_LAUNCH(0, 2, 2);
    } else if (kp == 160) NABO_TC_LAUNCH(10, 3, 0);
    else if (kp == 80) NABO_TC_LAUNCH(5, 3, 0);
    else NABO_TC_LAUNCH(0, 3, 0);
#undef NABO_TC_LAUNCH1
#undef NABO_TC_LAUNCH
    NABO_LAUNCH_CHECK("candidates_kernel");
    if (!overlap) tm.end(0);
    if (fused) {
        raw_out->buf = cbuf; raw_out->cnt = ccnt; raw_out->tau = ctau; raw_out->kprime = kprime;
        *cand_idx_out = cand; *kprime_out = kprime; *cert_tau_out = tau; *qn2_out = qn2; *scal_out = scal;
        *launches += 6;
        *n_split_io = 1;
        return 0;
    }
    if (raw_out) raw_out->buf = nullptr;
    if (pl.nq == 2) tc::emit_kernel<2><<<(unsigned)((n_slots + 7) / 8), 256, 0, st>>>(p);
    else tc::emit_kernel<3><<<(unsigned)((n_slots + 7) / 8), 256, 0, st>>>(p);
    NABO_LAUNCH_CHECK("emit_kernel");
    *launches += 1;
    if (n_split > 1) {
        int rc = nabo_tau_min_launch(tau, n_query, n_split, st);
        if (rc) return rc;
        *launches += 1;
    }
    *n_split_io = n_split;
    *cand_idx_out = cand; *kprime_out = kprime; *cert_tau_out = tau; *qn2_out = qn2; *scal_out = scal;
    *launches += 6;
    return 0;
}

#ifdef NABO_TC_STATS
extern "C" int nabo_dbg_tc_stats(unsigned long long* out_host, int reset) {
    cudaDeviceSynchronize();
    cudaMemcpyFromSymbol(out_host, tc::g_tc_stats, sizeof(unsigned long long) * 12);
    if (reset) { unsigned long long z[12] = {0}; cudaMemcpyToSymbol(tc::g_tc_stats, z, sizeof(z)); }
    return 0;
}
#endif

extern "C" int nabo_knn_candidates_width(int k, int drop_first) { return nabo_tc_kprime(k, drop_first); }

extern "C" size_t nabo_knn_candidates_workspace_bytes(int n_query, int n_ref, int g, int k, int drop_first) {
    return nabo_tc_workspace_bytes(n_query, n_ref, g, k, drop_first);
}

extern "C" int nabo_knn_candidates(const double* q, int ldq, const double* r, int ldr, int n_query, int n_ref, int g,
                                   int k, int metric, const uint8_t* ref_mask, int drop_first, int32_t* out_cand,
                                   float* out_tau, double* out_qn2, double* out_scal, void* workspace,
                                   size_t workspace_bytes, void* stream) {
    cudaStream_t st = (cudaStream_t)stream;
    NABO_ARG(metric == NABO_EUCLIDEAN || metric == NABO_COSINE, "candidates: metric %d has no tensor-core pass", metric);
    NABO_ARG(n_query >= 1 && n_ref >= 1 && ldq >= g && ldr >= g, "candidates: bad sizes");
    NABO_ARG(q && r && out_cand && out_tau, "candidates: null pointer");
    if (!nabo_tc_supported(g, k, drop_first))
        return nabo_set_error(NABO_EUNSUPPORTED, "candidates: g=%d k=%d outside the tensor-core tile plan", g, k);
    NaboArena ar(workspace, workspace_bytes);
    NaboStageTimer tm(false, st);
    int32_t* cand = nullptr;
    float* tau = nullptr;
    double *qn2 = nullptr, *scal = nullptr;
    int kprime = 0, launches = 0;
    int one_list = 0;
    int rc = nabo_tc_candidates(q, ldq, r, ldr, n_query, n_ref, g, k, metric, ref_mask, drop_first, &one_list, ar, &cand,
                                &kprime, &tau, &qn2, &scal, &launches, tm, st);
    if (rc) return rc;
    NABO_CUDA(cudaMemcpyAsync(out_cand, cand, sizeof(int32_t) * (size_t)n_query * kprime, cudaMemcpyDeviceToDevice, st));
    NABO_CUDA(cudaMemcpyAsync(out_tau, tau, sizeof(float) * (size_t)n_query, cudaMemcpyDeviceToDevice, st));
    if (out_qn2) NABO_CUDA(cudaMemcpyAsync(out_qn2, qn2, sizeof(double) * (size_t)n_query, cudaMemcpyDeviceToDevice, st));
    if (out_scal) NABO_CUDA(cudaMemcpyAsync(out_scal, scal, sizeof(double) * 4, cudaMemcpyDeviceToDevice, st));
    return 0;
}
```

Measured before the change: 22.99 million.

## Split only the tail wave of query items across SMs and merge pieces in rerank

Replaces the old uniform n_split of every query item with a schedule in which full waves of items run unsplit. Only the remainder items (fewer than the SM count) are split into reference-tile ranges spread over all SMs. Rerank then unions up to three candidate pieces per split row, using a shared threshold and a histogram cut. This targets the idle SMs in the last wave and removes the emit and tau-min kernels in the fused path. The cost is more complex scheduling, extra workspace, a memset, and a fallback to failed rows when the union overflows.

```diff
diff --git a/nabo_b200/csrc/exact.cu b/nabo_b200/csrc/exact.cu
--- a/nabo_b200/csrc/exact.cu
+++ b/nabo_b200/csrc/exact.cu
@@ -635,6 +635,76 @@
     return 0;
 }
 #endif
+__device__ __forceinline__ int split_union(const NaboCandBuf& cb, int qi, int lane, uint32_t* hist, float (&fv)[4],
+                                           uint32_t (&kpl)[4], float& tf) {
+    const int np = cb.pieces[qi / cb.rows_per_item];
+    const uint32_t ts = cb.shared_tau[qi];
+    tf = ts >= float_to_sortable(CUDART_INF_F) ? CUDART_INF_F : sortable_to_float(ts);
+    auto key_at = [&](int pc, int u, int& n_pc) {
+        const size_t row = (size_t)pc * cb.plane + qi;
+        n_pc = cb.cnt[row];
+        const int i = u * 32 + lane;
+        return i < n_pc ? cb.buf[row * sel::CAP + i] : 0ull;
+    };
+    int m = 0;
+    float flo = CUDART_INF_F, fhi = -CUDART_INF_F;
+    for (int pc = 0; pc < np; ++pc)
+#pragma unroll
+        for (int u = 0; u < 4; ++u) {
+            int n_pc;
+            const unsigned long long kv = key_at(pc, u, n_pc);
+            const float f = __uint_as_float((uint32_t)(kv >> 32));
+            if (u * 32 + lane < n_pc && f < tf) { ++m; flo = fminf(flo, f); fhi = fmaxf(fhi, f); }
+        }
+    m = __reduce_add_sync(0xffffffffu, m);
+    int cut_bin = 255;
+    float scale = 0.f;
+    if (m > sel::CAP) {
+        flo = sortable_to_float(__reduce_min_sync(0xffffffffu, float_to_sortable(flo)));
+        fhi = sortable_to_float(__reduce_max_sync(0xffffffffu, float_to_sortable(fhi)));
+        reinterpret_cast<uint4*>(hist)[lane * 2] = make_uint4(0, 0, 0, 0);
+        reinterpret_cast<uint4*>(hist)[lane * 2 + 1] = make_uint4(0, 0, 0, 0);
+        __syncwarp();
+        scale = fhi > flo ? 255.999f / (fhi - flo) : 0.f;
+        for (int pc = 0; pc < np; ++pc)
+#pragma unroll
+            for (int u = 0; u < 4; ++u) {
+                int n_pc;
+                const float f = __uint_as_float((uint32_t)(key_at(pc, u, n_pc) >> 32));
+                if (u * 32 + lane < n_pc && f < tf) atomicAdd(&hist[max(0, min(255, (int)((f - flo) * scale)))], 1u);
+            }
+        __syncwarp();
+        int kept;
+        sel::hist_cut(hist, m, lane, cb.kprime, cut_bin, kept);
+        __syncwarp();
+        if (kept > sel::CAP) return -1;
+    }
+    unsigned long long* stage = reinterpret_cast<unsigned long long*>(hist);
+    int base = 0;
+    for (int pc = 0; pc < np; ++pc)
+#pragma unroll
+        for (int u = 0; u < 4; ++u) {
+            int n_pc;
+            const unsigned long long kv = key_at(pc, u, n_pc);
+            const float f = __uint_as_float((uint32_t)(kv >> 32));
+            const bool keep = u * 32 + lane < n_pc && f < tf &&
+                              (m <= sel::CAP || max(0, min(255, (int)((f - flo) * scale))) <= cut_bin);
+            const unsigned mk = __ballot_sync(0xffffffffu, keep);
+            if (keep) stage[base + __popc(mk & ((1u << lane) - 1u))] = kv;
+            base += __popc(mk);
+        }
+    __syncwarp();
+#pragma unroll
+    for (int u = 0; u < 4; ++u) {
+        const int i = u * 32 + lane;
+        const unsigned long long kv = i < base ? stage[i] : 0ull;
+        fv[u] = __uint_as_float((uint32_t)(kv >> 32));
+        kpl[u] = (uint32_t)kv;
+    }
+    __syncwarp();
+    return base;
+}
+
 template <int METRIC, bool FROM_BUF>
 __global__ void __launch_bounds__(128)
 rerank_kernel(const double* __restrict__ q, int ldq, const double* __restrict__ r, int ldr, int n_query,
@@ -659,18 +729,28 @@
     int nc = 0;
     float tau_q = CUDART_INF_F;
     if (FROM_BUF) {
-        const int n = __ldcg(cb.cnt + qi);
-        const unsigned long long* gb = cb.buf + (size_t)qi * sel::CAP;
-        float fv[4];
+        uint32_t* hist = reinterpret_cast<uint32_t*>(smem + hist_off) + warp * 256;
+        const bool split_row = qi >= cb.split_row0;
+        float fv[4], tau_rest = CUDART_INF_F;
         uint32_t kpl[4];
-#pragma unroll
-        for (int u = 0; u < 4; ++u) {
-            const int i = u * 32 + lane;
-            const unsigned long long kv = i < n ? __ldcg(gb + i) : 0ull;
-            fv[u] = __uint_as_float((uint32_t)(kv >> 32));
-            kpl[u] = (uint32_t)kv;
-        }
-        uint32_t* hist = reinterpret_cast<uint32_t*>(smem + hist_off) + warp * 256;
+        int n;
+        if (!split_row) {
+            n = __ldcg(cb.cnt + qi);
+            const unsigned long long* gb = cb.buf + (size_t)qi * sel::CAP;
+#pragma unroll
+            for (int u = 0; u < 4; ++u) {
+                const int i = u * 32 + lane;
+                const unsigned long long kv = i < n ? __ldcg(gb + i) : 0ull;
+                fv[u] = __uint_as_float((uint32_t)(kv >> 32));
+                kpl[u] = (uint32_t)kv;
+            }
+        } else {
+            n = split_union(cb, qi, lane, hist, fv, kpl, tau_rest);
+            if (n < 0) {
+                if (lane == 0) fail_rows[atomicAdd(fail_count, 1)] = qi;
+                return;
+            }
+        }
         int bin[4], cut_bin, kept;
         bool reach;
         sel::histogram_cut(fv, n, lane, cb.kprime, hist, bin, cut_bin, kept, reach);
@@ -714,7 +794,7 @@
             }
             tmax = sortable_to_float(__reduce_max_sync(0xffffffffu, float_to_sortable(tmax)));
             nc = kept;
-            tau_q = reach ? tmax : __ldcg(cb.tau + qi);
+            tau_q = reach ? tmax : split_row ? tau_rest : __ldcg(cb.tau + qi);
         } else {
             uint32_t ks[4];
 #pragma unroll
@@ -723,7 +803,7 @@
             nc = n < cb.kprime ? n : cb.kprime;
             const int e = cb.kprime - 1;
             const uint32_t ts = __shfl_sync(0xffffffffu, (e >> 5) ? ks[1] : ks[0], e & 31);
-            tau_q = n >= cb.kprime ? sortable_to_float(ts) : __ldcg(cb.tau + qi);
+            tau_q = n >= cb.kprime ? sortable_to_float(ts) : split_row ? tau_rest : __ldcg(cb.tau + qi);
 #pragma unroll
             for (int u = 0; u < 2; ++u)
                 if (u * 32 + lane < nc) ix[u * 32 + lane] = (int)kpl[u];
@@ -848,7 +928,8 @@
     const bool vec2 = ((uintptr_t)r & 15) == 0 && (ldr & 1) == 0;
     dim3 grid((n_query - row0 + 3) / 4);
     NaboCandBuf cb;
-    cb.buf = nullptr; cb.cnt = nullptr; cb.tau = nullptr; cb.kprime = 0;
+    cb.buf = nullptr; cb.cnt = nullptr; cb.tau = nullptr; cb.kprime = 0; cb.split_row0 = n_query; cb.rows_per_item = 1;
+    cb.plane = 0; cb.pieces = nullptr; cb.shared_tau = nullptr;
     if (from_buf) {
         NABO_ARG(from_buf->kprime >= 1 && from_buf->kprime <= 64 && from_buf->kprime == n_cand,
                  "rerank: buffer mode needs K' = n_cand <= 64");
diff --git a/nabo_b200/csrc/fast.cu b/nabo_b200/csrc/fast.cu
--- a/nabo_b200/csrc/fast.cu
+++ b/nabo_b200/csrc/fast.cu
@@ -99,8 +99,6 @@
     int kprime = 0, launches = 0;
     NaboCandBuf raw;
     raw.buf = nullptr;
-    int n_split = nabo_tc_split(n_query, n_ref, g);
-    while (n_split > 1 && n_split * nabo_tc_kprime(k, drop_first) > 128) --n_split;
     int* fail_rows = ar.take<int>(n_query);
     int* fail_count = ar.take<int>(1);
     char* split_ws = ar.take<char>(nabo_exact_split_workspace(k + (drop_first ? 1 : 0)));
@@ -109,8 +107,8 @@
     NaboTailSplit tail;
     tail.rows_full = 0; tail.applies = 0;
     tail.dry = stats_host != nullptr;
-    int rc = nabo_tc_candidates(q, ldq, r, ldr, n_query, n_ref, g, k, metric, mask, drop_first, &n_split, ar, &cand,
-                                &kprime, &tau, &qn2, &scal, &launches, tm, st, &raw, &tail);
+    int rc = nabo_tc_candidates(q, ldq, r, ldr, n_query, n_ref, g, k, metric, mask, drop_first, ar, &cand, &kprime, &tau,
+                                &qn2, &scal, &launches, tm, st, &raw, &tail);
     if (rc) return rc;
     if (!ar.ok) return nabo_set_error(NABO_EWORKSPACE, "knn: workspace too small");
     NaboCert cert;
@@ -120,14 +118,14 @@
     int row0 = 0;
     if (tail.rows_full > 0) {
         rc = nabo_rerank_launch(q, ldq, r, ldr, tail.rows_full, n_ref, g, k, metric, f, mask, drop_first, idx_offset, cand,
-                                kprime * n_split, cert, fail_rows, fail_count, out_idx, out_dist, route, st, &raw, 0, true);
+                                kprime, cert, fail_rows, fail_count, out_idx, out_dist, route, st, &raw, 0, true);
         if (rc) return rc;
         tm.end(0);
         row0 = tail.rows_full;
     }
     launches += tail.applies;
     rc = nabo_rerank_launch(q, ldq, r, ldr, n_query, n_ref, g, k, metric, f, mask, drop_first, idx_offset, cand,
-                            kprime * n_split, cert, fail_rows, fail_count, out_idx, out_dist, route, st,
+                            kprime, cert, fail_rows, fail_count, out_idx, out_dist, route, st,
                             raw.buf ? &raw : nullptr, row0);
     if (rc) return rc;
     tm.end(1);
diff --git a/nabo_b200/csrc/knn_internal.cuh b/nabo_b200/csrc/knn_internal.cuh
--- a/nabo_b200/csrc/knn_internal.cuh
+++ b/nabo_b200/csrc/knn_internal.cuh
@@ -66,6 +66,11 @@
     const int* cnt;
     const float* tau;
     int kprime;
+    int split_row0;
+    int rows_per_item;
+    size_t plane;
+    const int* pieces;
+    const unsigned int* shared_tau;
 };
 int nabo_rerank_launch(const double* q, int ldq, const double* r, int ldr, int n_query, int n_ref, int g, int k,
                        int metric, double f, const uint8_t* mask, int drop_first, int idx_offset,
@@ -84,9 +89,8 @@
 int nabo_tc_kprime(int k, int drop_first);
 size_t nabo_tc_workspace_bytes(int n_query, int n_ref, int g, int k, int drop_first);
 #define NABO_TC_MAX_SPLIT 3
-int nabo_tc_split(int n_query, int n_ref, int g);
 int nabo_tc_candidates(const double* q, int ldq, const double* r, int ldr, int n_query, int n_ref, int g, int k,
-                       int metric, const uint8_t* mask, int drop_first, int* n_split_io, NaboArena& ar, int32_t** cand_idx_out,
+                       int metric, const uint8_t* mask, int drop_first, NaboArena& ar, int32_t** cand_idx_out,
                        int* kprime_out, float** cert_tau_out, double** qn2_out, double** scal_out, int* launches,
                        NaboStageTimer& tm, cudaStream_t st, NaboCandBuf* raw_out = nullptr, NaboTailSplit* tail = nullptr);
 
diff --git a/nabo_b200/csrc/select.cuh b/nabo_b200/csrc/select.cuh
--- a/nabo_b200/csrc/select.cuh
+++ b/nabo_b200/csrc/select.cuh
@@ -159,6 +159,39 @@
     __syncwarp();
 }
 
+__device__ __forceinline__ bool hist_cut(const uint32_t* hist, int n, int lane, int kprime, int& cut_bin, int& kept) {
+    const uint4 h0 = reinterpret_cast<const uint4*>(hist)[lane * 2];
+    const uint4 h1 = reinterpret_cast<const uint4*>(hist)[lane * 2 + 1];
+    const uint32_t c[8] = {h0.x, h0.y, h0.z, h0.w, h1.x, h1.y, h1.z, h1.w};
+    uint32_t mine = 0;
+#pragma unroll
+    for (int e = 0; e < 8; ++e) mine += c[e];
+    uint32_t incl = mine;
+#pragma unroll
+    for (int o = 1; o < 32; o <<= 1) {
+        const uint32_t v = __shfl_up_sync(0xffffffffu, incl, o);
+        if (lane >= o) incl += v;
+    }
+    const unsigned reach = __ballot_sync(0xffffffffu, incl >= (uint32_t)kprime);
+    cut_bin = 255;
+    kept = n;
+    if (reach) {
+        const int owner = __ffs(reach) - 1;
+        uint32_t run = incl - mine;
+        int b = 7;
+        uint32_t k_at = 0;
+        bool found = false;
+#pragma unroll
+        for (int e = 0; e < 8; ++e) {
+            run += c[e];
+            if (!found && run >= (uint32_t)kprime) { found = true; b = e; k_at = run; }
+        }
+        cut_bin = __shfl_sync(0xffffffffu, lane * 8 + b, owner);
+        kept = (int)__shfl_sync(0xffffffffu, k_at, owner);
+    }
+    return reach != 0;
+}
+
 __device__ __forceinline__ void histogram_cut(const float (&fv)[KPL], int n, int lane, int kprime, uint32_t* hist,
                                               int (&bin)[KPL], int& cut_bin, int& kept, bool& reach_out) {
     float flo = CUDART_INF_F, fhi = -CUDART_INF_F;
@@ -178,37 +211,8 @@
         if (u * 32 + lane < n) atomicAdd(&hist[bin[u]], 1u);
     }
     __syncwarp();
-    const uint4 h0 = reinterpret_cast<const uint4*>(hist)[lane * 2];
-    const uint4 h1 = reinterpret_cast<const uint4*>(hist)[lane * 2 + 1];
-    const uint32_t c[8] = {h0.x, h0.y, h0.z, h0.w, h1.x, h1.y, h1.z, h1.w};
-    uint32_t mine = 0;
-#pragma unroll
-    for (int e = 0; e < 8; ++e) mine += c[e];
-    uint32_t incl = mine;
-#pragma unroll
-    for (int o = 1; o < 32; o <<= 1) {
-        const uint32_t v = __shfl_up_sync(0xffffffffu, incl, o);
-        if (lane >= o) incl += v;
-    }
-    const unsigned reach = __ballot_sync(0xffffffffu, incl >= (uint32_t)kprime);
-    cut_bin = 255;
-    kept = n;
-    reach_out = reach != 0;
-    if (reach) {
-        const int owner = __ffs(reach) - 1;
-        uint32_t run = incl - mine;
-        int b = 7;
-        uint32_t k_at = 0;
-        bool found = false;
-#pragma unroll
-        for (int e = 0; e < 8; ++e) {
-            run += c[e];
-            if (!found && run >= (uint32_t)kprime) { found = true; b = e; k_at = run; }
-        }
-        cut_bin = __shfl_sync(0xffffffffu, lane * 8 + b, owner);
-        kept = (int)__shfl_sync(0xffffffffu, k_at, owner);
-    }
-    __syncwarp();
-}
-
-}
+    reach_out = hist_cut(hist, n, lane, kprime, cut_bin, kept);
+    __syncwarp();
+}
+
+}
diff --git a/nabo_b200/csrc/tc_candidates.cu b/nabo_b200/csrc/tc_candidates.cu
--- a/nabo_b200/csrc/tc_candidates.cu
+++ b/nabo_b200/csrc/tc_candidates.cu
@@ -197,15 +197,36 @@
     if (IS_QUERY && c == 0 && live && qn2_out) qn2_out[row] = n2_row;
 }
 
+constexpr int MIN_PIECE = 32;
+struct Tail {
+    long long units;
+    int rtiles, grid, s;
+    __host__ __device__ long long bound(int c) const {
+        if (c >= grid) return units;
+        if (s > 0) {
+            if ((long long)c >= units / rtiles * s) return units;
+            return (long long)(c / s) * rtiles + (long long)rtiles * (c % s) / s;
+        }
+        long long b = units * c / grid;
+        const int off = (int)(b % rtiles);
+        if (off < MIN_PIECE) b -= off;
+        else if (off > rtiles - MIN_PIECE) b += rtiles - off;
+        return b;
+    }
+};
+
 struct Params {
     const __half* qa;
     const __half* rb;
     int n_query, n_ref, kp, n_items, n_rtiles, stages, kprime, kc_out, soft;
-    int signal_round;
-    int n_split;
+    int n_full;
+    int signal;
+    Tail tail;
     unsigned long long* cand_buf;
     int* cand_cnt;
     float* cand_tau;
+    unsigned int* shared_tau;
+    int* pieces;
     int32_t* cand_idx;
     float* cert_tau;
     size_t a_off, b_off, sort_off, bar_off;
@@ -221,13 +242,15 @@
 using namespace sel;
 
 #ifdef NABO_TC_STATS
-__device__ unsigned long long g_tc_stats[12];
+constexpr int NSTAT = 13;
+__device__ unsigned long long g_tc_stats[NSTAT];
 #define TC_STAT(i, v) (tc_loc[i] += (unsigned long long)(v))
 #define TC_CLK(var) const long long var = clock64()
 #define TC_CLK_ADD(i, t0) (tc_loc[i] += (unsigned long long)(clock64() - (t0)))
-#define TC_DECL unsigned long long tc_loc[12] = {0, 0, 0, 0, 0, 0, 0, 0, 0, 0, 0, 0}
-#define TC_FLUSH do { if ((threadIdx.x & 31) == 0) for (int i_ = 0; i_ < 12; ++i_) { if (tc_loc[i_]) atomicAdd(&g_tc_stats[i_], tc_loc[i_]); tc_loc[i_] = 0; } } while (0)
-#define TC_ARG , unsigned long long (&tc_loc)[12]
+#define TC_DECL unsigned long long tc_loc[NSTAT] = {}
+#define TC_FLUSH do { if ((threadIdx.x & 31) == 0) for (int i_ = 0; i_ < NSTAT; ++i_) { if (tc_loc[i_]) atomicAdd(&g_tc_stats[i_], tc_loc[i_]); tc_loc[i_] = 0; } } while (0)
+#define TC_SPLIT_MOVE do { tc_loc[11] += tc_loc[3]; tc_loc[12] += tc_loc[4]; tc_loc[3] = tc_loc[4] = 0; } while (0)
+#define TC_ARG , unsigned long long (&tc_loc)[NSTAT]
 #define TC_PASS , tc_loc
 #else
 #define TC_STAT(i, v)
@@ -235,6 +258,7 @@
 #define TC_CLK_ADD(i, t0)
 #define TC_DECL
 #define TC_FLUSH
+#define TC_SPLIT_MOVE
 #define TC_ARG
 #define TC_PASS
 #endif
@@ -280,18 +304,23 @@
 }
 
 template <bool SPLIT>
-__device__ __forceinline__ bool work_piece(const Params& p, int c, int r, int& slot, int& qitem, int& j0, int& j1) {
-    slot = c + r * (int)gridDim.x;
-    if (!SPLIT) {
-        if (slot >= p.n_items) return false;
-        qitem = slot; j0 = 0; j1 = p.n_rtiles;
+__device__ __forceinline__ bool work_piece(const Params& p, int c, int r, int& item, int& j0, int& j1) {
+    const int slot = c + r * (int)gridDim.x;
+    if (slot < p.n_full) {
+        item = slot; j0 = 0; j1 = p.n_rtiles;
         return true;
     }
-    if (slot >= p.n_items * p.n_split) return false;
-    qitem = slot / p.n_split;
-    const int seg = slot - qitem * p.n_split;
-    j0 = (int)((long long)p.n_rtiles * seg / p.n_split);
-    j1 = (int)((long long)p.n_rtiles * (seg + 1) / p.n_split);
+    if (!SPLIT) return false;
+    int k = r - p.n_full / (int)gridDim.x;
+    const long long rt = p.n_rtiles, lo = p.tail.bound(c), hi = p.tail.bound(c + 1);
+    const long long s1 = (lo / rt + 1) * rt;
+    if (k < 2 && s1 < hi && s1 + rt >= hi && s1 - lo < hi - s1) k = 1 - k;
+    const long long start = k == 0 ? lo : (lo / rt + k) * rt;
+    if (start >= hi) return false;
+    const long long i = start / rt;
+    item = p.n_full + (int)i;
+    j0 = (int)(start - i * rt);
+    j1 = (int)((hi < (i + 1) * rt ? hi : (i + 1) * rt) - i * rt);
     return true;
 }
 
@@ -324,8 +353,8 @@
         if (lane == 0) {
             uint32_t t = 0, it = 0;
             for (int wr = 0;; ++wr, ++it) {
-                int w, item, j0, j1;
-                if (!work_piece<SPLIT>(p, blockIdx.x, wr, w, item, j0, j1)) break;
+                int item, j0, j1;
+                if (!work_piece<SPLIT>(p, blockIdx.x, wr, item, j0, j1)) break;
                 ptx::mbar_wait_hint(&bars->a_empty, (it & 1) ^ 1, SLEEP_NS);
                 ptx::mbar_arrive_expect_tx(&bars->a_full, NQ * a_tile_bytes);
                 for (int q = 0; q < NQ; ++q) {
@@ -355,8 +384,8 @@
             const uint64_t bd0 = ptx::make_smem_desc(ptx::smem_u32(smem + p.b_off), lbo, sbo);
             uint32_t t = 0, it = 0, n = 0;
             for (int wr = 0;; ++wr, ++it) {
-                int w, item, j0, j1;
-                if (!work_piece<SPLIT>(p, blockIdx.x, wr, w, item, j0, j1)) break;
+                int item, j0, j1;
+                if (!work_piece<SPLIT>(p, blockIdx.x, wr, item, j0, j1)) break;
                 ptx::mbar_wait(&bars->a_full, it & 1);
                 for (int j = j0; j < j1; ++j, n += NQ, ++t)
                     for (int sl = 0; sl < nslab; ++sl) {
@@ -410,11 +439,10 @@
         uint32_t t = 0;
         uint32_t* hist = reinterpret_cast<uint32_t*>(smem + p.sort_off) + (size_t)warp * 256;
         TC_DECL;
-        for (int wr = 0;; ++wr) {
-            int w, item, j0, j1;
-            if (!work_piece<SPLIT>(p, blockIdx.x, wr, w, item, j0, j1)) break;
-            unsigned long long* mybuf = p.cand_buf + ((size_t)w * NQ * TILE + slot) * CAP;
-            float tau = CUDART_INF_F;
+        auto sweep = [&](auto shared_tag, int j0, int j1, size_t bi, unsigned int* stau) {
+            constexpr bool SHARED = decltype(shared_tag)::value;
+            unsigned long long* mybuf = p.cand_buf + bi * CAP;
+            float tau = SHARED ? fminf(CUDART_INF_F, sortable_to_float(__ldcg(stau))) : CUDART_INF_F;
             int cnt = 0;
             TC_CLK(t_item);
             for (int j = j0; j < j1; ++j, ++t) {
@@ -437,7 +465,11 @@
                         int nc;
                         float nt;
                         compact_select(gb, n, lane, p.kprime, p.soft - 8, hist, nc, nt);
-                        if (lane == src) { cnt = nc; tau = nt; }
+                        if (lane == src) {
+                            cnt = nc;
+                            if (!SHARED) tau = nt;
+                            else if (nt < tau) { tau = nt; atomicMin(stau, float_to_sortable(nt)); }
+                        }
                         if (lane == 0) TC_STAT(4, 1);
                     }
                     TC_CLK_ADD(5, t_c);
@@ -461,15 +493,38 @@
                 }
             }
             TC_CLK(t_e);
-            p.cand_cnt[(size_t)w * NQ * TILE + slot] = cnt;
-            p.cand_tau[(size_t)w * NQ * TILE + slot] = tau;
+            p.cand_cnt[bi] = cnt;
+            p.cand_tau[bi] = tau;
             TC_CLK_ADD(9, t_e);
             TC_CLK_ADD(10, t_item);
+            if (SHARED) TC_SPLIT_MOVE;
             TC_FLUSH;
-            if (!SPLIT && p.signal_round == wr + 1) {
+        };
+        for (int wr = 0;; ++wr) {
+            int item, j0, j1;
+            if (!work_piece<false>(p, blockIdx.x, wr, item, j0, j1)) break;
+            sweep(std::integral_constant<bool, false>(), j0, j1, (size_t)item * NQ * TILE + slot, nullptr);
+        }
+        if (SPLIT) {
+            if (p.signal) {
                 __threadfence();
                 asm volatile("bar.sync 1, %0;" ::"n"(N_EPI_WARPS * 32) : "memory");
                 if (threadIdx.x == 0) asm volatile("griddepcontrol.launch_dependents;" ::: "memory");
+            }
+            const size_t plane = (size_t)p.n_items * NQ * TILE;
+            for (int wr = p.n_full / (int)gridDim.x;; ++wr) {
+                int item, j0, j1;
+                if (!work_piece<true>(p, blockIdx.x, wr, item, j0, j1)) break;
+                int piece = 0;
+                if (j0 > 0) {
+                    const long long s0 = (long long)(item - p.n_full) * p.n_rtiles;
+                    piece = 1;
+                    for (int d = (int)blockIdx.x - 1; d >= 0 && p.tail.bound(d) > s0; --d) ++piece;
+                }
+                NABO_DEV_ASSERT(piece < NABO_TC_MAX_SPLIT);
+                const size_t qrow = (size_t)item * NQ * TILE + slot;
+                sweep(std::integral_constant<bool, true>(), j0, j1, piece * plane + qrow, p.shared_tau + qrow);
+                if (j1 == p.n_rtiles && threadIdx.x == 0) p.pieces[item] = piece + 1;
             }
         }
     }
@@ -482,29 +537,25 @@
 __global__ void __launch_bounds__(256)
 emit_kernel(const Params p) {
     const int lane = threadIdx.x & 31;
-    const long long wq = (long long)blockIdx.x * 8 + (threadIdx.x >> 5);
-    if (wq >= (long long)p.n_items * p.n_split * NQ * TILE) return;
-    const int w = (int)(wq / (NQ * TILE)), slot = (int)(wq - (long long)w * NQ * TILE);
-    const int item = w / p.n_split, seg = w - item * p.n_split;
-    const long long qg = (long long)item * NQ * TILE + slot;
+    const long long qg = (long long)blockIdx.x * 8 + (threadIdx.x >> 5);
     if (qg >= p.n_query) return;
-    const int n = p.cand_cnt[wq];
-    const float old_tau = p.cand_tau[wq];
+    const int n = p.cand_cnt[qg];
+    const float old_tau = p.cand_tau[qg];
     NABO_DEV_ASSERT(n >= 0 && n <= CAP);
     uint32_t ks[KPL], kpl[KPL];
     int nc;
     float nt;
-    compact_sort_inline(p.cand_buf + (size_t)wq * CAP, n, lane, p.kprime, ks, kpl, nc, nt);
+    compact_sort_inline(p.cand_buf + (size_t)qg * CAP, n, lane, p.kprime, ks, kpl, nc, nt);
 #pragma unroll
     for (int u = 0; u < 4; ++u) {
         const int i = u * 32 + lane;
         if (i < p.kc_out) {
             int32_t id = -1;
             if (i < nc && kpl[u] < (uint32_t)p.n_ref) id = (int32_t)kpl[u];
-            p.cand_idx[(qg * p.n_split + seg) * p.kc_out + i] = id;
-        }
-    }
-    if (lane == 0) p.cert_tau[(long long)seg * p.n_query + qg] = n >= p.kprime ? nt : old_tau;
+            p.cand_idx[qg * p.kc_out + i] = id;
+        }
+    }
+    if (lane == 0) p.cert_tau[qg] = n >= p.kprime ? nt : old_tau;
 }
 
 }
@@ -523,21 +574,26 @@
     return kprime;
 }
 
-static int tc_grid(int n_items) {
+static int tc_sms() {
     int dev = 0, sms = 148;
     cudaGetDevice(&dev);
     cudaDeviceGetAttribute(&sms, cudaDevAttrMultiProcessorCount, dev);
-    return n_items < sms ? n_items : sms;
-}
-
-int nabo_tc_split(int n_query, int n_ref, int g) {
-    const int nq = tc::plan_smem(g).nq;
-    const int n_items = (n_query + nq * tc::TILE - 1) / (nq * tc::TILE);
-    const int n_rtiles = (n_ref + tc::TILE - 1) / tc::TILE;
-    int s = n_items > 0 ? tc_grid(1 << 30) / n_items : 1;
-    if (s > NABO_TC_MAX_SPLIT) s = NABO_TC_MAX_SPLIT;
-    while (s > 1 && n_rtiles / s < 32) --s;
-    return s < 1 ? 1 : s;
+    return sms;
+}
+
+static tc::Tail tail_schedule(int rem, int n_rtiles, int grid) {
+    tc::Tail t;
+    t.units = (long long)rem * n_rtiles;
+    t.rtiles = n_rtiles;
+    t.grid = grid;
+    t.s = 0;
+    if (t.units / grid < (n_rtiles + 1) / 2) {
+        int s = rem > 0 ? grid / rem : 1;
+        if (s > NABO_TC_MAX_SPLIT) s = NABO_TC_MAX_SPLIT;
+        while (s > 1 && n_rtiles / s < tc::MIN_PIECE) --s;
+        t.s = s < 1 ? 1 : s;
+    }
+    return t;
 }
 
 __global__ void tau_min_kernel(float* __restrict__ tau, int n_query, int n_split) {
@@ -561,23 +617,24 @@
     const int n_items = (n_query + nq * tc::TILE - 1) / (nq * tc::TILE);
     const int n_rtiles = (n_ref + tc::TILE - 1) / tc::TILE;
     const int kprime = nabo_tc_kprime(k, drop_first);
+    const size_t rows = (size_t)n_items * nq * tc::TILE;
     size_t b = 0;
     b += nabo_align_up((size_t)n_items * nq * tb, 256);
     b += nabo_align_up((size_t)n_rtiles * tb, 256);
     b += nabo_align_up((size_t)n_query * 8, 256) * 2;
     b += nabo_align_up((size_t)n_ref * 8, 256);
-    b += nabo_align_up((size_t)n_items * NABO_TC_MAX_SPLIT * nq * tc::TILE * (tc::CAP * 8 + 8), 256) + 512;
-    b += nabo_align_up((size_t)n_query * kprime * 4 * NABO_TC_MAX_SPLIT, 256);
-    b += nabo_align_up((size_t)n_query * 4 * NABO_TC_MAX_SPLIT, 256) + nabo_align_up((size_t)n_query * 4, 256);
+    b += nabo_align_up(rows * NABO_TC_MAX_SPLIT * (tc::CAP * 8 + 8), 256) + 512;
+    b += nabo_align_up(rows * 4, 256) + nabo_align_up((size_t)n_items * 4, 256);
+    b += nabo_align_up((size_t)n_query * kprime * 4, 256);
+    b += nabo_align_up((size_t)n_query * 4, 256) * 2;
     b += 4096;
     return b;
 }
 
 int nabo_tc_candidates(const double* q, int ldq, const double* r, int ldr, int n_query, int n_ref, int g, int k,
-                       int metric, const uint8_t* mask, int drop_first, int* n_split_io, NaboArena& ar, int32_t** cand_idx_out,
+                       int metric, const uint8_t* mask, int drop_first, NaboArena& ar, int32_t** cand_idx_out,
                        int* kprime_out, float** cert_tau_out, double** qn2_out, double** scal_out, int* launches,
                        NaboStageTimer& tm, cudaStream_t st, NaboCandBuf* raw_out, NaboTailSplit* tail) {
-    int n_split = *n_split_io;
     const int kp = tc::kp_for(g);
     const tc::SmemPlan pl = tc::plan_smem(g);
     const size_t tb = tc::tile_bytes(kp);
@@ -585,25 +642,31 @@
     const int n_qtiles = n_items * pl.nq;
     const int n_rtiles = (n_ref + tc::TILE - 1) / tc::TILE;
     const int kprime = nabo_tc_kprime(k, drop_first);
-    if (n_split < 1 || n_split > NABO_TC_MAX_SPLIT) n_split = 1;
-    const int grid = tc_grid(n_items * n_split);
+    const bool fused = raw_out && kprime <= 64;
+    const int sms = tc_sms();
+    const int n_full = fused ? n_items / sms * sms : n_items;
+    const bool split = n_full < n_items;
+    const int grid = split || n_items > sms ? sms : n_items;
 
     __half* qa = (__half*)ar.take<char>((size_t)n_qtiles * tb);
     __half* rb = (__half*)ar.take<char>((size_t)n_rtiles * tb);
     double* qnorm = ar.take<double>(n_query);
     double* qn2 = ar.take<double>(n_query);
     double* rnorm = ar.take<double>(n_ref);
-    const size_t n_slots = (size_t)n_items * n_split * pl.nq * tc::TILE;
-    unsigned long long* cbuf = ar.take<unsigned long long>(n_slots * tc::CAP);
-    int* ccnt = ar.take<int>(n_slots);
-    float* ctau = ar.take<float>(n_slots);
-    int32_t* cand = ar.take<int32_t>((size_t)n_query * kprime * n_split);
-    float* tau = ar.take<float>((size_t)n_query * n_split);
+    const size_t rows = (size_t)n_items * pl.nq * tc::TILE;
+    unsigned long long* cbuf = ar.take<unsigned long long>(rows * (split ? NABO_TC_MAX_SPLIT : 1) * tc::CAP);
+    int* ccnt = ar.take<int>(rows * (split ? NABO_TC_MAX_SPLIT : 1));
+    float* ctau = ar.take<float>(rows * (split ? NABO_TC_MAX_SPLIT : 1));
+    unsigned int* stau = split ? ar.take<unsigned int>(rows) : nullptr;
+    int* pieces = split ? ar.take<int>(n_items) : nullptr;
+    int32_t* cand = fused ? nullptr : ar.take<int32_t>((size_t)n_query * kprime);
+    float* tau = fused ? nullptr : ar.take<float>(n_query);
     double* scal = ar.take<double>(4);
     unsigned int* maxbits = ar.take<unsigned int>(2);
     if (!ar.ok) return nabo_set_error(NABO_EWORKSPACE, "knn: workspace too small for the tensor-core pass");
 
     NABO_CUDA(cudaMemsetAsync(maxbits, 0, 2 * sizeof(unsigned int), st));
+    if (split) NABO_CUDA(cudaMemsetAsync(stau, 0xff, rows * sizeof(unsigned int), st));
     tc::norms_kernel<<<(n_query + 255) / 256, 256, 0, st>>>(q, ldq, n_query, g, qnorm, maxbits);
     tc::norms_kernel<<<(n_ref + 255) / 256, 256, 0, st>>>(r, ldr, n_ref, g, rnorm, maxbits + 1);
     tc::scale_kernel<<<1, 1, 0, st>>>(maxbits, maxbits + 1, metric == NABO_COSINE ? 1 : 0, scal);
@@ -615,18 +678,19 @@
     tc::Params p;
     p.qa = qa; p.rb = rb;
     p.n_query = n_query; p.n_ref = n_ref; p.kp = kp; p.n_items = n_items; p.n_rtiles = n_rtiles;
-    p.stages = pl.stages; p.kprime = kprime; p.kc_out = kprime; p.n_split = n_split;
-    p.cand_buf = cbuf; p.cand_cnt = ccnt; p.cand_tau = ctau; p.cand_idx = cand; p.cert_tau = tau;
+    p.stages = pl.stages; p.kprime = kprime; p.kc_out = kprime;
+    p.n_full = n_full;
+    p.tail = tail_schedule(n_items - n_full, n_rtiles, grid);
+    p.cand_buf = cbuf; p.cand_cnt = ccnt; p.cand_tau = ctau; p.shared_tau = stau; p.pieces = pieces;
+    p.cand_idx = cand; p.cert_tau = tau;
     p.a_off = pl.a_off; p.b_off = pl.b_off; p.sort_off = pl.sort_off; p.bar_off = pl.bar_off;
     p.soft = tc::CAP - tc::CHUNK - 16 > kprime ? tc::CAP - tc::CHUNK - 16 : kprime;
-    const bool fused = raw_out && n_split == 1 && kprime <= 64;
-    const int rem_items = n_items % grid;
-    const bool tail_applies = tail && fused && n_items > grid && rem_items > 0 && grid - rem_items >= 16;
+    const bool tail_applies = tail && split && n_full > 0;
     const bool overlap = tail_applies && !tail->dry;
-    p.signal_round = overlap ? n_items / grid : 0;
+    p.signal = overlap ? 1 : 0;
     if (tail) {
         tail->applies = tail_applies ? 1 : 0;
-        tail->rows_full = overlap ? (n_items - rem_items) * pl.nq * tc::TILE : 0;
+        tail->rows_full = overlap ? n_full * pl.nq * tc::TILE : 0;
     }
 #define NABO_TC_LAUNCH1(KS, SPLIT, NQ, SLAB)                                                                       \
     do {                                                                                                           \
@@ -636,7 +700,7 @@
     } while (0)
 #define NABO_TC_LAUNCH(KS, NQ, SLAB)                                                                               \
     do {                                                                                                           \
-        if (n_split > 1) NABO_TC_LAUNCH1(KS, true, NQ, SLAB);                                                      \
+        if (split) NABO_TC_LAUNCH1(KS, true, NQ, SLAB);                                                            \
         else NABO_TC_LAUNCH1(KS, false, NQ, SLAB);                                                                 \
     } while (0)
     if (pl.stages < 2) return nabo_set_error(NABO_EUNSUPPORTED, "knn: g=%d outside the tensor-core tile plans", g);
@@ -650,34 +714,31 @@
 #undef NABO_TC_LAUNCH
     NABO_LAUNCH_CHECK("candidates_kernel");
     if (!overlap) tm.end(0);
+    *kprime_out = kprime; *qn2_out = qn2; *scal_out = scal;
+    *launches += 6;
     if (fused) {
         raw_out->buf = cbuf; raw_out->cnt = ccnt; raw_out->tau = ctau; raw_out->kprime = kprime;
-        *cand_idx_out = cand; *kprime_out = kprime; *cert_tau_out = tau; *qn2_out = qn2; *scal_out = scal;
-        *launches += 6;
-        *n_split_io = 1;
+        raw_out->split_row0 = split ? n_full * pl.nq * tc::TILE : n_query;
+        raw_out->rows_per_item = pl.nq * tc::TILE;
+        raw_out->plane = rows;
+        raw_out->pieces = pieces; raw_out->shared_tau = stau;
+        *cand_idx_out = nullptr; *cert_tau_out = nullptr;
         return 0;
     }
     if (raw_out) raw_out->buf = nullptr;
-    if (pl.nq == 2) tc::emit_kernel<2><<<(unsigned)((n_slots + 7) / 8), 256, 0, st>>>(p);
-    else tc::emit_kernel<3><<<(unsigned)((n_slots + 7) / 8), 256, 0, st>>>(p);
+    if (pl.nq == 2) tc::emit_kernel<2><<<(unsigned)((n_query + 7) / 8), 256, 0, st>>>(p);
+    else tc::emit_kernel<3><<<(unsigned)((n_query + 7) / 8), 256, 0, st>>>(p);
     NABO_LAUNCH_CHECK("emit_kernel");
     *launches += 1;
-    if (n_split > 1) {
-        int rc = nabo_tau_min_launch(tau, n_query, n_split, st);
-        if (rc) return rc;
-        *launches += 1;
-    }
-    *n_split_io = n_split;
-    *cand_idx_out = cand; *kprime_out = kprime; *cert_tau_out = tau; *qn2_out = qn2; *scal_out = scal;
-    *launches += 6;
+    *cand_idx_out = cand; *cert_tau_out = tau;
     return 0;
 }
 
 #ifdef NABO_TC_STATS
 extern "C" int nabo_dbg_tc_stats(unsigned long long* out_host, int reset) {
     cudaDeviceSynchronize();
-    cudaMemcpyFromSymbol(out_host, tc::g_tc_stats, sizeof(unsigned long long) * 12);
-    if (reset) { unsigned long long z[12] = {0}; cudaMemcpyToSymbol(tc::g_tc_stats, z, sizeof(z)); }
+    cudaMemcpyFromSymbol(out_host, tc::g_tc_stats, sizeof(unsigned long long) * tc::NSTAT);
+    if (reset) { unsigned long long z[tc::NSTAT] = {0}; cudaMemcpyToSymbol(tc::g_tc_stats, z, sizeof(z)); }
     return 0;
 }
 #endif
@@ -704,9 +765,8 @@
     float* tau = nullptr;
     double *qn2 = nullptr, *scal = nullptr;
     int kprime = 0, launches = 0;
-    int one_list = 0;
-    int rc = nabo_tc_candidates(q, ldq, r, ldr, n_query, n_ref, g, k, metric, ref_mask, drop_first, &one_list, ar, &cand,
-                                &kprime, &tau, &qn2, &scal, &launches, tm, st);
+    int rc = nabo_tc_candidates(q, ldq, r, ldr, n_query, n_ref, g, k, metric, ref_mask, drop_first, ar, &cand, &kprime,
+                                &tau, &qn2, &scal, &launches, tm, st);
     if (rc) return rc;
     NABO_CUDA(cudaMemcpyAsync(out_cand, cand, sizeof(int32_t) * (size_t)n_query * kprime, cudaMemcpyDeviceToDevice, st));
     NABO_CUDA(cudaMemcpyAsync(out_tau, tau, sizeof(float) * (size_t)n_query, cudaMemcpyDeviceToDevice, st));
```

After: 22.32 million (median of 6 runs). 0.971x the previous value.
